# mitrefireline/simfire

Measured on AMD Instinct MI355X. Metric: cell-updates/sec (grid x envs x steps), higher is better.
Workload: dtype u8 status + u8 sprite masks + f64 burn_amounts

## Files before the change

### simfire_amd/csrc/sf_run_kernels.h

```cpp
#pragma once

#include "sf_common.h"
#include "sf_step_kernels.h"

namespace {

constexpr int kMarkDw = 32;
constexpr int kStripDw = 19;
#ifdef SF_NO_PERM_ELIG
#define ELIG(x) elig01(x)
#else
#define ELIG(x) elig01_perm(x)
#endif
constexpr int kRunCtl = 24;
constexpr int kRunMaxD = 4;

typedef uint32_t __attribute__((aligned(1))) u32_unaligned;
typedef uint32_t u32x4 __attribute__((ext_vector_type(4)));

__host__ __device__ inline size_t win_lds_bytes(int n_waves)
{
    const int WR = n_waves * 4;
    return (size_t)WR * 64 * 8 + 8 * 8 * 4 + 128 * 4 + 64 * 4 + (size_t)(WR + 2) * 18 * 4 + (size_t)WR * 16 + (size_t)2 * WR * 64 * 2 + (size_t)2 * WR * 64 +
           (size_t)WR * 64 + (size_t)WR * 8 + 256 * 4;
}
__host__ __device__ inline size_t run_strip_dwords(int n_waves)
{
    const size_t strips = (size_t)n_waves * (64 * kStripDw + kMarkDw), win = (win_lds_bytes(n_waves) + 15) / 16 * 4;
    return strips > win ? strips : win;
}

__host__ __device__ inline size_t run_lds_bytes(const Geo &g, int n_waves, int vcap, int team = 0, int team_rcap = 0)
{
    const int maps = (team || g.VW == 1) ? 4 : 1;
    const int rows = team && team_rcap ? team_rcap + 2 : g.H;
    size_t b = (size_t)maps * rows * g.VW * 8 + (size_t)vcap * 4 + run_strip_dwords(n_waves) * 4 + kRunCtl * 4;
    if (team) b += (size_t)2 * g.PV * 16 + 64 * 4;
#ifdef SF_PHASES
    b += 16 * 16 * 4;
#endif
    return b;
}

}
#include "sf_win_kernels.h"
namespace {

struct RunEnv {
    uint8_t *cells;
    double *burn;
    uint32_t *settled;
    const double *rt;
    unsigned long long *vb;
    unsigned long long *vf, *vl;
    uint8_t *tdirty;
    int32_t *tot;
};

struct WalkCell {
    bool cand;
    uint32_t yx;
    uint32_t own_spost;
    uint32_t owed;
    double bn, r_tab;
};

template <int ATT, int CNT = 0>
__device__ __forceinline__ WalkAcc run_walk(const StepArgs &a, const RunEnv &ev, const Masks &mk, int complete,
                                            uint32_t lo_mask, uint32_t hi_mask, const uint32_t *strips,
                                            uint32_t pend, int lane, int th_log, PhaseClock &pc,
                                            uint32_t excl, uint32_t w16, uint4 s7)
{
    const Geo &g = a.g;
    WalkAcc acc = {0u, 0u, 0u, 0u};
    auto front = [&](uint32_t j, int own) {
        WalkCell c;
        const bool valid = j < pend;
        const int jl = own;
        const uint32_t base = (uint32_t)__builtin_amdgcn_ds_bpermute(jl << 2, (int)excl);
        const uint32_t wl = (uint32_t)__builtin_amdgcn_ds_bpermute(jl << 2, (int)w16);
        int b = 0;
        {
            uint32_t r = valid ? j - base : 0u, x = wl & 0xFFFFu, n;
            n = (uint32_t)__popc(x & 0xFFu); if (r >= n) { r -= n; b += 8; x >>= 8; }
            n = (uint32_t)__popc(x & 0xFu); if (r >= n) { r -= n; b += 4; x >>= 4; }
            n = (uint32_t)__popc(x & 0x3u); if (r >= n) { r -= n; b += 2; x >>= 2; }
            if (r >= (x & 1u)) b += 1;
            b &= 15;
        }
        uint32_t s_post = 0;
        const bool on_line = valid && ((wl >> (16 + b)) & 1u);
        if (__ballot(on_line) != 0ull) {
            const uint32_t d0 = (uint32_t)__builtin_amdgcn_ds_bpermute(jl << 2, (int)s7.x), d1 = (uint32_t)__builtin_amdgcn_ds_bpermute(jl << 2, (int)s7.y);
            const uint32_t d2 = (uint32_t)__builtin_amdgcn_ds_bpermute(jl << 2, (int)s7.z), d3 = (uint32_t)__builtin_amdgcn_ds_bpermute(jl << 2, (int)s7.w);
            const uint32_t dd = (b >> 2) == 0 ? d0 : ((b >> 2) == 1 ? d1 : ((b >> 2) == 2 ? d2 : d3));
            if (on_line) s_post = (dd >> (8 * (b & 3))) & 7u;
        }
        const uint32_t *rec = strips + jl * kStripDw;
        const uint32_t hdr = rec[0];
        const int y = hdr & 0xFFFF, x = (int)(hdr >> 16) * 16 + b;
        const uint32_t idx = (uint32_t)(y * g.P + x);
        const int q = (3 + b) >> 2;
        const uint32_t sh = (uint32_t)(3 + b) & 3u;
        uint32_t u0 = rec[1 + q], u1 = rec[2 + q], m0 = rec[7 + q], m1 = rec[8 + q], d0 = rec[13 + q], d1 = rec[14 + q];
        asm volatile("" : "+v"(u0), "+v"(u1), "+v"(m0), "+v"(m1), "+v"(d0), "+v"(d1));
        const uint32_t up3 = __builtin_amdgcn_alignbyte(u1, u0, sh);
        const uint32_t mid3 = __builtin_amdgcn_alignbyte(m1, m0, sh);
        const uint32_t dn3 = __builtin_amdgcn_alignbyte(d1, d0, sh);
        const int bestk = pick_winner8(up3, mid3, dn3, mk, lo_mask, hi_mask);
        c.cand = valid && bestk >= 0;
        c.yx = (uint32_t)y | ((uint32_t)x << 16);
        c.own_spost = ((mid3 >> 8) & 0xFFu) | (s_post << 8);
        c.owed = 0; c.bn = 0.0; c.r_tab = 0.0;
        {
            const unsigned long long cb = __ballot(c.cand);
            acc.n_active += (uint32_t)__popcll(cb);
            acc.cand |= cb != 0ull;
        }
        if (c.cand) {
            c.bn = ev.burn[idx];
            c.r_tab = ev.rt[(uint32_t)bestk * (uint32_t)(g.H * g.P) + idx];
            if (ATT && s_post >= SF_FIRELINE) c.owed = (uint32_t)complete - ev.settled[idx];
        }
        return c;
    };
    auto back = [&](const WalkCell &c) {
        bool ignited = false;
        if (c.cand) {
            const int y = (int)(c.yx & 0xFFFFu), x = (int)(c.yx >> 16);
            const uint32_t idx = (uint32_t)(y * g.P + x), s_post = c.own_spost >> 8;
            const bool line = s_post >= SF_FIRELINE;
            double bn = c.bn;
            double ros = c.r_tab * g.update_rate;
            if (line) {
                if (ATT) {
                    const double f = line_factor(s_post);
                    bn = lazy_sub(bn, f, c.owed);
                    ros = ros - f;
                    ev.settled[idx] = (uint32_t)complete + 1u;
                } else ros = 0.0;
            }
            bn = bn + ros;
            ev.burn[idx] = bn;
            if (bn > g.pixel_scale) {
                ignited = true;
                const uint8_t nb = (uint8_t)(((c.own_spost & 0xFFu) & ~mk.b_clr) | mk.b_new);
#ifdef SF_STORE_ORDER_WAIT
                asm volatile("s_waitcnt vmcnt(0)" ::: "memory");
#endif
                uint8_t *cell = ev.cells + bl_cell(g, y, x);
                cell[kBlStatus] = (uint8_t)SF_BURNING;
                cell[0] = nb;
                const int bw = y * g.VW + (x >> 10);
                atomicOr(&ev.vb[bw], 1ull << ((x >> 4) & 63));
                if (ev.vf) {
                    if ((x & 15) == 0) atomicOr(&ev.vf[bw], 1ull << ((x >> 4) & 63));
                    if ((x & 15) == 15) atomicOr(&ev.vl[bw], 1ull << ((x >> 4) & 63));
                }
                ev.tdirty[(y >> th_log) * g.TX + ((x >> 4) >> g.logLC)] = 1;
                if (CNT && line) { atomicAdd(ev.tot + s_post, -1); atomicAdd(ev.tot + SF_UNBURNED, 1); }
            }
        }
        acc.n_ignite += (uint32_t)__popcll(__ballot(ignited));
    };
    for (uint32_t j0 = 0; j0 < pend; j0 += 128) {
        const bool two = j0 + 64 < pend;
        int own0 = 0, own1 = 0;
        {
            uint8_t *marks = reinterpret_cast<uint8_t *>(const_cast<uint32_t *>(strips) + 64 * kStripDw);
            reinterpret_cast<uint16_t *>(marks)[lane] = 0;
            const uint32_t mine_n = (uint32_t)__popc(w16 & 0xFFFFu);
            if (mine_n && excl < j0 + 128u && excl + mine_n > j0) marks[excl < j0 ? 0u : excl - j0] = (uint8_t)(lane + 1);
            __builtin_amdgcn_fence(__ATOMIC_RELEASE, "wavefront");
            __builtin_amdgcn_wave_barrier();
            __builtin_amdgcn_fence(__ATOMIC_ACQUIRE, "wavefront");
            const uint32_t m0 = wave_scan_max(marks[lane]);
            own0 = (int)((m0 - 1u) & 63u);
            if (two) {
                const uint32_t carry = wave_last(m0);
                const uint32_t m1 = wave_scan_max(marks[64 + lane]);
                own1 = (int)(((m1 > carry ? m1 : carry) - 1u) & 63u);
            }
        }
        WalkCell c0 = front(j0 + (uint32_t)lane, own0), c1;
        c1.cand = false; c1.yx = 0; c1.own_spost = 0; c1.owed = 0; c1.bn = 0.0; c1.r_tab = 0.0;
        if (two) c1 = front(j0 + 64u + (uint32_t)lane, own1);
        pc.mark(7);
        asm volatile("" : "+v"(c0.bn), "+v"(c0.r_tab), "+v"(c0.owed), "+v"(c1.bn), "+v"(c1.r_tab), "+v"(c1.owed));
        back(c0);
        if (two) back(c1);
        pc.mark(8);
    }
    __builtin_amdgcn_fence(__ATOMIC_RELEASE, "wavefront");
    __builtin_amdgcn_wave_barrier();
    __builtin_amdgcn_fence(__ATOMIC_ACQUIRE, "wavefront");
    pc.mark(9);
    return acc;
}

struct JoinArgs { uint32_t *xj; unsigned long long *xcut; uint32_t *xerr; int E, t_cap, team_recut, join_floor, join_ovh, join_local; unsigned long long team_timeout; };
__device__ __forceinline__ uint4 find_team(const JoinArgs a, uint32_t *sc)
{
    typedef unsigned long long u64;
    const int tid = threadIdx.x, wave = tid >> 6, lane = tid & 63, n_waves = blockDim.x >> 6, nthr = blockDim.x;
    const int E = a.E;
    const uint4 none = make_uint4(0xFFFFFFFFu, 0, 0, 0);
    const uint32_t my_xcc = (uint32_t)__builtin_amdgcn_s_getreg((20 << 0) | (0 << 6) | (31 << 11)) & 15u;
    const unsigned long long t_start = __builtin_amdgcn_s_memrealtime();
    __syncthreads();
    for (;;) {
        uint32_t best = 0, best_e = 0;
        for (int i = tid; i < E; i += nthr) {
            const uint32_t cnt = __hip_atomic_load(a.xj + i, __ATOMIC_RELAXED, __HIP_MEMORY_SCOPE_AGENT);
            const uint32_t b = __hip_atomic_load(a.xj + E + i, __ATOMIC_RELAXED, __HIP_MEMORY_SCOPE_AGENT);
            const long long c = cnt & 0xFFFFu;
            if ((cnt & kJoinClosed) || !b || c >= a.t_cap || c == 0) continue;
            if (a.join_local && __hip_atomic_load(a.xj + 2 * E + 2 + i, __ATOMIC_RELAXED, __HIP_MEMORY_SCOPE_AGENT) != my_xcc) continue;
            const long long per = (long long)(b >> 14) << 4, left = b & 0x3FFFu;
            if (left <= 2 * a.team_recut) continue;
            const long long share_now = per / c, share_join = per / (c + 1);
            const long long now_t = c == 1 ? per : (share_now > a.join_floor ? share_now : a.join_floor) + a.join_ovh;
            const long long join_t = (share_join > a.join_floor ? share_join : a.join_floor) + a.join_ovh;
            if (join_t * 8 >= now_t * 7) continue;
            const long long fin = (now_t * left) >> 8;
            const uint32_t score = fin > 0xFFFFFFFFll ? 0xFFFFFFFFu : (fin < 1 ? 1u : (uint32_t)fin);
            if (score > best) { best = score; best_e = (uint32_t)i; }
        }
        const uint32_t wm = wave_umax(best);
        const int src = __ffsll((long long)__ballot(best == wm)) - 1;
        const uint32_t we = (uint32_t)__builtin_amdgcn_readlane((int)best_e, src);
        if (lane == 0) { sc[wave * 2] = wm; sc[wave * 2 + 1] = we; }
        __syncthreads();
        uint32_t bs = 0, be = 0;
        for (int w = 0; w < n_waves; ++w) { const uint32_t v = sc[2 * w]; if (v > bs) { bs = v; be = sc[2 * w + 1]; } }
        if (tid == 0 && bs == 0) sc[40] = __hip_atomic_load(a.xj + 2 * E, __ATOMIC_RELAXED, __HIP_MEMORY_SCOPE_AGENT);
        __syncthreads();
        if (bs == 0) {
            const uint32_t closed = sc[40];
            __syncthreads();
            if (closed >= (uint32_t)E) return none;
            if (__builtin_amdgcn_s_memrealtime() - t_start > a.team_timeout) return none;
            for (int q = 0; q < 8; ++q) __builtin_amdgcn_s_sleep(127);
            continue;
        }
        if (tid == 0) {
            uint32_t res = 0xFFFFFFFFu;
            const uint32_t old = atomicAdd(a.xj + be, 1u);
            if (!(old & kJoinClosed) && (old & 0xFFFFu) < (uint32_t)a.t_cap) {
                const uint32_t idx = old & 0xFFFFu;
                const unsigned long long t0 = __builtin_amdgcn_s_memrealtime();
                for (;;) {
                    const u64 x = __hip_atomic_load(a.xcut + be, __ATOMIC_RELAXED, __HIP_MEMORY_SCOPE_AGENT);
                    if (x == ~0ull) break;
                    if ((uint32_t)((x >> 24) & 0xFFu) > idx) { res = idx; sc[42] = (uint32_t)((x >> 24) & 0xFFu); sc[43] = (uint32_t)(x & 0xFFFFFFu); break; }
                    __builtin_amdgcn_s_sleep(16);
                    if (__builtin_amdgcn_s_memrealtime() - t0 > a.team_timeout) {
                        *reinterpret_cast<volatile uint32_t *>(a.xerr) = 1u;
                        res = 0xFFFFFFFEu;
                        break;
                    }
                }
            }
            sc[41] = res;
        }
        __syncthreads();
        const uint32_t res = sc[41], tn = sc[42], s0 = sc[43];
        __syncthreads();
        if (res == 0xFFFFFFFEu) return none;
        if (res == 0xFFFFFFFFu) continue;
        __builtin_amdgcn_fence(__ATOMIC_ACQUIRE, "agent");
        return make_uint4(be, res, tn, s0);
    }
}

template <int OFF>
__device__ __forceinline__ uint32_t kernarg_line(const void *ka)
{
    uint32_t d;
    asm volatile("s_load_dword %0, %1, %2" : "=s"(d) : "s"(ka), "n"(OFF));
    return d;
}
template <int BYTES>
__device__ __forceinline__ void kernarg_touch()
{
    const void *ka = (const void *)__builtin_amdgcn_kernarg_segment_ptr();
    uint32_t d0 = 0, d1 = 0, d2 = 0, d3 = 0, d4 = 0, d5 = 0, d6 = 0, d7 = 0, d8 = 0, d9 = 0, d10 = 0, d11 = 0, d12 = 0, d13 = 0, d14 = 0, d15 = 0;
    static_assert(BYTES <= 16 * 64, "more lines than this touches");
    d0 = kernarg_line<0>(ka);
    if (BYTES > 1 * 64) d1 = kernarg_line<1 * 64>(ka);
    if (BYTES > 2 * 64) d2 = kernarg_line<2 * 64>(ka);
    if (BYTES > 3 * 64) d3 = kernarg_line<3 * 64>(ka);
    if (BYTES > 4 * 64) d4 = kernarg_line<4 * 64>(ka);
    if (BYTES > 5 * 64) d5 = kernarg_line<5 * 64>(ka);
    if (BYTES > 6 * 64) d6 = kernarg_line<6 * 64>(ka);
    if (BYTES > 7 * 64) d7 = kernarg_line<7 * 64>(ka);
    if (BYTES > 8 * 64) d8 = kernarg_line<8 * 64>(ka);
    if (BYTES > 9 * 64) d9 = kernarg_line<9 * 64>(ka);
    if (BYTES > 10 * 64) d10 = kernarg_line<10 * 64>(ka);
    if (BYTES > 11 * 64) d11 = kernarg_line<11 * 64>(ka);
    if (BYTES > 12 * 64) d12 = kernarg_line<12 * 64>(ka);
    if (BYTES > 13 * 64) d13 = kernarg_line<13 * 64>(ka);
    if (BYTES > 14 * 64) d14 = kernarg_line<14 * 64>(ka);
    if (BYTES > 15 * 64) d15 = kernarg_line<15 * 64>(ka);
    asm volatile("s_waitcnt lgkmcnt(0)" : "+s"(d0), "+s"(d1), "+s"(d2), "+s"(d3), "+s"(d4), "+s"(d5), "+s"(d6), "+s"(d7), "+s"(d8), "+s"(d9), "+s"(d10), "+s"(d11), "+s"(d12),
                 "+s"(d13), "+s"(d14), "+s"(d15));
}

template <int MAXD, int ATT, int DIAG, int MIT, int TEAM = 0>
__global__ __launch_bounds__(1024) void k_run(StepArgs a_by_value, const int n_steps_launch, int vcap, int bsz)
{
    kernarg_touch<(int)sizeof(StepArgs) + 12>();
#ifdef SF_ARGS_BY_VALUE
    constexpr bool kArgsByValue = true;
#else
    constexpr bool kArgsByValue = TEAM == 2 || MIT == -2 || (MIT == 0 && TEAM == 0) || (TEAM == 1 && MAXD == 2);
#endif
    const StepArgs &a = kArgsByValue ? a_by_value : *(const StepArgs *)__builtin_amdgcn_kernarg_segment_ptr();
    extern __shared__ uint4 s_dyn[];
    const Geo &g = a.g;
    const int tid = threadIdx.x, wave = tid >> 6, lane = tid & 63, n_waves = blockDim.x >> 6, nthr = blockDim.x;
    int e_ = 0, tm_ = 0, tn_ = 1;
    bool no_work = false;
    if (TEAM) {
        const uint32_t tt = a.team_tab[blockIdx.x];
        if (tt == kTeamUnused) { if (TEAM != 2) return; no_work = true; }
        else { e_ = (int)(tt & 0xFFFFu); tm_ = (int)((tt >> 16) & 0xFFu); tn_ = (int)(tt >> 24); }
    } else if (a.todo_cnt) {
        const uint32_t n_left = *a.todo_cnt;
        if (blockIdx.x >= n_left) return;
        e_ = (int)a.todo_list[blockIdx.x];
    } else e_ = a.order ? (int)a.order[blockIdx.x] : (int)blockIdx.x;
    int j_s0 = -1;
    for (bool first_pass = true;; first_pass = false) {
    if (TEAM == 2 && (!first_pass || no_work)) {
        if (a.team_recut >= n_steps_launch) return;
        uint32_t *sc = reinterpret_cast<uint32_t *>(s_dyn);
        JoinArgs ja;
        ja.xj = a.xj; ja.xcut = a.xcut; ja.xerr = a.xerr; ja.E = g.E; ja.team_recut = a.team_recut; ja.join_floor = a.join_floor; ja.join_ovh = a.join_ovh;
        ja.team_timeout = a.team_timeout; ja.join_local = a.join_local; ja.t_cap = kTeamMax < g.TY ? kTeamMax : g.TY;
        const uint4 t = find_team(ja, sc);
        if (t.x == 0xFFFFFFFFu) return;
        e_ = __builtin_amdgcn_readfirstlane((int)t.x); tm_ = __builtin_amdgcn_readfirstlane((int)t.y);
        tn_ = __builtin_amdgcn_readfirstlane((int)t.z); j_s0 = __builtin_amdgcn_readfirstlane((int)t.w);
    }
    {
    int n_steps = n_steps_launch;
    const int e = e_, tm = tm_;
    int tn = tn_;
    const unsigned long long clk0 = __builtin_readcyclecounter();
    const bool fine = TEAM ? true : (MAXD == 1 ? true : g.VW == 1);
    const int VW = MAXD == 1 ? 1 : g.VW;
    const int32_t *const mit = MIT == 0 ? nullptr : a.mit;
    const bool diag = DIAG > 0 ? true : g.diag != 0;
    const int lds_rows = TEAM && a.team_rcap ? a.team_rcap + 2 : g.H;
    unsigned long long *vb0 = reinterpret_cast<unsigned long long *>(s_dyn);
    uint32_t *vlist = reinterpret_cast<uint32_t *>(vb0 + (size_t)(fine ? 4 : 1) * lds_rows * VW);
    uint32_t *strips = vlist + vcap + wave * (64 * kStripDw + kMarkDw);
    uint32_t *ctl = vlist + vcap + run_strip_dwords(n_waves);
#ifdef SF_PHASES
    uint4 *halo = reinterpret_cast<uint4 *>(ctl + kRunCtl + 16 * 16);
#else
    uint4 *halo = reinterpret_cast<uint4 *>(ctl + kRunCtl);
#endif
    uint32_t *tcnt = reinterpret_cast<uint32_t *>(halo + 2 * g.PV);

    constexpr bool kWinPre = (MIT == 0 || MIT == -1) && MAXD == 1 && TEAM == 0;
    constexpr bool kWinAny = ((MIT == 0 && MAXD <= 2) || (MIT == -1 && MAXD == 1 && TEAM == 0 && DIAG == 1)) && TEAM != 2;
    constexpr bool kWinAdvice = kWinAny && !(MAXD == 1 && TEAM == 0);
    unsigned long long pre_w = 0ull, hint_v = 0ull;
    int32_t todo_v = 0;
    EnvState st;
    {
        typedef uint32_t u32x2v __attribute__((ext_vector_type(2)));
        const EnvState *const ps = a.commit + e;
        const bool want_pre = kWinPre && a.win && tid < g.H, want_hint = kWinAdvice && a.win && a.win_hint, want_todo = a.todo != nullptr;
        const void *const p_pre = want_pre ? (const void *)(a.vbits + (long long)e * g.vb_env + tid) : (const void *)ps;
        const void *const p_hint = want_hint ? (const void *)(a.win_hint + e) : (const void *)ps;
        const void *const p_todo = want_todo ? (const void *)(a.todo + e) : (const void *)ps;
        u32x2v v_pre, v_hint, v_hi;
        u32x4 v_lo;
        uint32_t v_todo;
        asm volatile("global_load_dwordx2 %0, %5, off\n\tglobal_load_dwordx2 %1, %6, off\n\tglobal_load_dword %2, %7, off\n\t"
                     "global_load_dwordx4 %3, %8, off\n\tglobal_load_dwordx2 %4, %8, off offset:16\n\ts_waitcnt vmcnt(0)"
                     : "=&v"(v_pre), "=&v"(v_hint), "=&v"(v_todo), "=&v"(v_lo), "=&v"(v_hi)
                     : "v"(p_pre), "v"(p_hint), "v"(p_todo), "v"(ps)
                     : "memory");
        if (want_pre) pre_w = (unsigned long long)v_pre.x | ((unsigned long long)v_pre.y << 32);
        if (want_hint) hint_v = (unsigned long long)v_hint.x | ((unsigned long long)v_hint.y << 32);
        if (want_todo) todo_v = (int32_t)v_todo;
        st.running = __builtin_amdgcn_readfirstlane((int)v_lo.x); st.steps = __builtin_amdgcn_readfirstlane((int)v_lo.y);
        st.complete = __builtin_amdgcn_readfirstlane((int)v_lo.z); st.time_quit = __builtin_amdgcn_readfirstlane((int)v_lo.w);
        st.elapsed = __hiloint2double(__builtin_amdgcn_readfirstlane((int)v_hi.y), __builtin_amdgcn_readfirstlane((int)v_hi.x));
    }
    const unsigned long long hint_pre = (unsigned long long)(uint32_t)__builtin_amdgcn_readfirstlane((int)(uint32_t)hint_v) | ((unsigned long long)(uint32_t)__builtin_amdgcn_readfirstlane((int)(uint32_t)(hint_v >> 32)) << 32);
    if (a.todo) n_steps = __builtin_amdgcn_readfirstlane(todo_v);
    if ((!st.running && !mit) || n_steps < 0) n_steps = 0;
    if (!TEAM && a.todo && a.todo_skip && n_steps == 0) return;
    unsigned long long *vb_glob = a.vbits + (long long)e * g.vb_env;
    const int n_words = g.H * VW;
    if (tid < kRunCtl) ctl[tid] = 0;
    const int th_log = 31 - __builtin_clz((unsigned)(g.LR * g.RB));
    uint32_t n_active = 0, n_ignite = 0, n_items_acc = 0, n_phase2 = 0, n_vec_done = 0;
    constexpr bool kWin = ((MIT == 0 && MAXD <= 2) || (MIT == -1 && MAXD == 1 && TEAM == 0 && DIAG == 1)) && TEAM != 2;
    constexpr int kWinGen = (MAXD == 1 && TEAM == 0) ? 0 : 1;
    constexpr int kWinMit = MIT == -1 ? 1 : 0;
    int32_t px = 0, py = 0, pty = 0;
    int s_begin = 0;
    bool win_result = false;
    PhaseClock wpc;
    const bool win_mit_ok = !kWinMit || !mit || a.mit_k <= 64;
    if (kWinMit && mit && a.mit_k <= 64 && n_steps > 0 && wave == n_waves - 1 && lane < a.mit_k) {
        const int32_t *p0 = mit + ((long long)e * a.mit_k + lane) * 3;
        px = p0[0]; py = p0[1]; pty = p0[2];
    }
    if (kWin && (!TEAM || tn == 1) && win_mit_ok && j_s0 < 0) {
        WinEnv we;
        we.cells = a.cells + (long long)e * g.cells_env;
        we.burn = a.burn + (long long)e * g.plane_env;
        we.settled = a.settled ? a.settled + (long long)e * g.plane_env : nullptr;
        we.rtc = a.rtc ? a.rtc + (long long)e * g.rt_env : nullptr;
        we.tdirty = a.tdirty + (long long)e * g.TY * g.TX;
        we.thist = a.thist + (long long)e * g.TY * g.TX * 8;
        we.vb_glob = vb_glob;
        we.vb_plane = (long long)g.E * g.vb_env;
        wpc.start();
#ifdef SF_PHASES
        wpc.tl = (e == g_timeline_env && g_timeline_step == -1) ? g_timeline + wave * 64 : nullptr;
#endif
        wpc.note(30);
        we.pre_w = pre_w; we.pre = kWinPre; we.hint = hint_pre;
        s_begin = run_window<ATT, kWinGen, kWinMit>(a, we, st, n_steps, diag, vlist + vcap, ctl, th_log, n_active, n_ignite, n_vec_done, wpc, e, win_result,
                                                    kWinMit ? mit : nullptr, n_steps, &px, &py, &pty, vlist, vcap >= 1024 ? 15 : 11);
        if (a.counters && tid == 0 && s_begin)
            atomicAdd(a.counters + (size_t)((blockIdx.x * 16) & (kCounterShards - 1)) * kCounterRow + 8, (unsigned long long)s_begin);
    }
    if (TEAM == 2 && j_s0 >= 0) s_begin = j_s0;
    const bool general = !kWin || (TEAM && tn > 1) || (s_begin < n_steps && (st.running || mit));
    if (TEAM == 0 && kWin && MIT == 0 && !general) {
#ifdef SF_PHASES
        if (lane == 0 && g_wave_log_launch == -2 && e < 4096) {
            if (wave == 0) { g_wave_log[e * 4 + 0] = __builtin_readcyclecounter() - clk0; g_wave_log[e * 4 + 2] = (unsigned long long)st.steps; }
            atomicAdd(&g_wave_log[e * 4 + 1], (unsigned long long)n_vec_done);
        }
#endif
        wpc.note(35);
        if (tid == 0) {
            a.commit[e] = st;
            if (a.cost) {
                const unsigned long long c = (__builtin_readcyclecounter() - clk0) >> 4;
                a.cost[e] = c > 0x0FFFFFFFull ? 0x0FFFFFFFu : (uint32_t)c;
            }
        }
        wpc.note(49);
        if (a.counters && lane == 0) {
            unsigned long long *cs = a.counters + (size_t)((blockIdx.x * 16 + wave) & (kCounterShards - 1)) * kCounterRow;
            if (n_active) atomicAdd(&cs[0], (unsigned long long)n_active);
            if (n_ignite) atomicAdd(&cs[1], (unsigned long long)n_ignite);
            if (n_vec_done) atomicAdd(&cs[5], (unsigned long long)n_vec_done);
        }
        if (a.res_block && !win_result && !(a.row_valid && n_steps == 0 && !mit)) {
            __syncthreads();
            counts_env(g, e, a.status, a.cells, a.tdirty, a.thist, st.running, st.steps, st.elapsed, a.res_block, a.res_elapsed, a.res_sink,
                       reinterpret_cast<int32_t (*)[6]>(vlist + vcap));
        }
        return;
    }
    int R0 = 0, R1 = g.H;
    auto cut_bands = [&](int steps_ahead) -> bool {
        int tid = threadIdx.x;
        asm volatile("" : "+v"(tid));
        const int lane = tid & 63, wave = tid >> 6;
        const int th = g.LR * g.RB, ntr = (g.H + th - 1) / th;
        if (tid < 64) tcnt[tid] = 0;
        __syncthreads();
        for (int y = tid; y < g.H; y += nthr) {
            uint32_t c = 0;
            for (int w = 0; w < VW; ++w) c += (uint32_t)__popcll(vb_glob[y * VW + w]);
            if (c) atomicAdd(&tcnt[y / th], c);
        }
        __syncthreads();
        if (wave == 0) {
            const uint32_t ci = lane < ntr ? tcnt[lane] : 0u;
            const uint32_t incl = wave_scan_incl(ci, lane), total = wave_last(incl);
            const unsigned long long nzb = __ballot(ci != 0u);
            int lo = 0, hi = ntr;
            if (a.team_rcap && nzb && !mit) {
                const int mt = (steps_ahead + 1 + th - 1) / th + 1;
                lo = __ffsll((long long)nzb) - 1 - mt; hi = 64 - __clzll((long long)nzb) + mt;
                lo = lo < 0 ? 0 : lo; hi = hi > ntr ? ntr : hi;
                if (hi - lo < tn) { hi = lo + tn < ntr ? lo + tn : ntr; lo = hi - tn > 0 ? hi - tn : 0; }
            }
            const int cap = a.team_rcap ? a.team_rcap / th : ntr;
            if (a.team_rcap && !nzb && !mit) hi = ntr < cap * tn ? ntr : cap * tn;
            int cut[kTeamMax + 1];
            cut[0] = lo; cut[tn] = hi;
            for (int j = 1; j < tn; ++j) {
                const unsigned long long bal = __ballot(lane < ntr && (unsigned long long)incl * (unsigned)tn >= (unsigned long long)total * (unsigned)j);
                int c = total ? __ffsll((long long)bal) : lo + (hi - lo) * j / tn;
                if (c < cut[j - 1] + 1) c = cut[j - 1] + 1;
                if (c > cut[j - 1] + cap) c = cut[j - 1] + cap;
                cut[j] = c;
            }
            for (int j = tn - 1; j >= 1; --j) {
                if (cut[j] > cut[j + 1] - 1) cut[j] = cut[j + 1] - 1;
                if (cut[j] < cut[j + 1] - cap) cut[j] = cut[j + 1] - cap;
            }
            bool fits = true;
            for (int j = 0; j < tn; ++j) fits = fits && cut[j + 1] - cut[j] >= 1 && cut[j + 1] - cut[j] <= cap;
            if (lane == 0) { tcnt[0] = (uint32_t)(cut[tm] * th); tcnt[1] = (uint32_t)(cut[tm + 1] * th); tcnt[2] = fits ? 1u : 0u; }
        }
        __syncthreads();
        R0 = (int)tcnt[0]; R1 = (int)tcnt[1];
        const bool fits = __builtin_amdgcn_readfirstlane((int)tcnt[2]) != 0;
        R0 = __builtin_amdgcn_readfirstlane(R0); R1 = __builtin_amdgcn_readfirstlane(R1);
        if (R1 > g.H) R1 = g.H;
        __syncthreads();
        return fits;
    };
    {
        bool fits = true;
        if (TEAM && (tn > 1 || a.team_rcap) && general) fits = cut_bands(tn > 1 && a.team_recut > 0 && a.team_recut < n_steps ? a.team_recut : n_steps - s_begin);
        if (TEAM && a.todo_out && tm == 0 && tid == 0) a.todo_out[e] = fits ? 0 : n_steps - s_begin;
        if (TEAM && !fits) {
            if (!a.todo_out && tid == 0) *reinterpret_cast<volatile uint32_t *>(a.xerr) = 1u;
            if (s_begin > 0 && tm == 0 && tid == 0) a.commit[e] = st;
            return;
        }
    }
    bool has_up = TEAM && tm > 0, has_dn = TEAM && tm + 1 < tn;
    if (TEAM == 2 && tm == 0 && j_s0 < 0 && tid == 0)
        __hip_atomic_store(a.xj + 2 * g.E + 2 + e, (uint32_t)__builtin_amdgcn_s_getreg((20 << 0) | (0 << 6) | (31 << 11)) & 15u, __ATOMIC_RELAXED, __HIP_MEMORY_SCOPE_AGENT);
    auto team_release = [&]() {
        if (TEAM == 2 && a.join_local == 1) asm volatile("s_waitcnt vmcnt(0)" ::: "memory");
        else __builtin_amdgcn_fence(__ATOMIC_RELEASE, "agent");
    };
    auto team_acquire = [&]() { __builtin_amdgcn_fence(__ATOMIC_ACQUIRE, "agent"); };
    bool one_l2 = false;
    bool gave_up = false;
    auto line_up = [&](const uint32_t tag, const bool report) {
        typedef unsigned long long u64;
        int lane = threadIdx.x & 63;
        asm volatile("" : "+v"(lane));
        const uint32_t xcc = (uint32_t)__builtin_amdgcn_s_getreg((20 << 0) | (0 << 6) | (31 << 11)) & 15u;
        if (lane == 0) __hip_atomic_store(a.xg + ((size_t)e * kTeamMax + tm) * 3 + 2, ((u64)tag << 32) | (u64)xcc, __ATOMIC_RELAXED, __HIP_MEMORY_SCOPE_AGENT);
        u64 x = ((u64)tag << 32) | xcc;
        const unsigned long long t0 = __builtin_amdgcn_s_memrealtime();
        for (;;) {
            if (lane < tn) x = __hip_atomic_load(a.xg + ((size_t)e * kTeamMax + lane) * 3 + 2, __ATOMIC_RELAXED, __HIP_MEMORY_SCOPE_AGENT);
            if (__all((uint32_t)(x >> 32) >= tag)) break;
            __builtin_amdgcn_s_sleep(2);
            if (gave_up || __builtin_amdgcn_s_memrealtime() - t0 > a.team_timeout) {
                if (report) {
                    if (lane == 0) *reinterpret_cast<volatile uint32_t *>(a.xerr) = 1u;
                    gave_up = true;
                }
                break;
            }
        }
        one_l2 = __all((uint32_t)(x >> 32) >= tag && ((uint32_t)x & 15u) == xcc) && !a.team_far;
    };
    unsigned long long *vb = vb0, *vf = nullptr, *vl = nullptr, *ve = nullptr;
    auto load_band = [&]() {
        int tid = threadIdx.x;
        asm volatile("" : "+v"(tid));
        const int yoff = TEAM && a.team_rcap ? R0 - 1 : 0;
        vb = vb0 - (long long)yoff * VW;
        vf = fine ? vb + (size_t)lds_rows * VW : nullptr; vl = fine ? vb + (size_t)2 * lds_rows * VW : nullptr;
        ve = fine ? vb + (size_t)3 * lds_rows * VW : nullptr;
        const int y_lo = TEAM && a.team_rcap ? (R0 > 0 ? R0 - 1 : 0) : 0, y_hi = TEAM && a.team_rcap ? (R1 < g.H ? R1 + 1 : g.H) : g.H;
        for (int i = y_lo * VW + tid; i < y_hi * VW; i += nthr) {
            vb[i] = vb_glob[i];
            if (fine) {
                vf[i] = vb_glob[(long long)g.E * g.vb_env + i];
                vl[i] = vb_glob[2ll * g.E * g.vb_env + i];
                ve[i] = ~0ull;
            }
        }
        if (TEAM && tn > 1) {
            for (int i = tid; i < 2 * g.PV; i += nthr) {
                const int side = i >= g.PV, v = side ? i - g.PV : i, yh = side ? R1 : R0 - 1;
                uint4 r = make_uint4(0, 0, 0, 0);
                if (side ? has_dn : has_up)
                    r = *reinterpret_cast<const uint4 *>(a.cells + (long long)e * g.cells_env + bl_vec(g, yh, v) + (yh & 1) * 16);
                halo[i] = r;
            }
        }
    };
    if (general) load_band();
    PhaseClock pc;
#ifdef SF_PHASES
    uint32_t *ph_acc = ctl + kRunCtl + wave * 16;
    if (lane < 16) ph_acc[lane] = 0;
    pc.start(ph_acc);
#else
    pc.start();
#endif
    __syncthreads();
    if (TEAM == 1 && tn > 1) {
        if (tid == 0) {
            uint32_t *w = a.xdone + g.E + e;
            constexpr uint32_t kGo = 0x40000000u, kAbort = 0x80000000u, kDecided = 0xC0000000u;
            auto decide = [&](uint32_t bit) -> uint32_t {
                for (;;) {
                    uint32_t cur = __hip_atomic_load(w, __ATOMIC_RELAXED, __HIP_MEMORY_SCOPE_AGENT);
                    if (cur & kDecided) return cur & kDecided;
                    if (__hip_atomic_compare_exchange_strong(w, &cur, cur | bit, __ATOMIC_RELAXED, __ATOMIC_RELAXED, __HIP_MEMORY_SCOPE_AGENT)) return bit;
                }
            };
            const uint32_t mine = __hip_atomic_fetch_add(w, 1u, __ATOMIC_RELAXED, __HIP_MEMORY_SCOPE_AGENT) + 1u;
            uint32_t d = mine & kDecided;
            if (!d && (mine & 0xFFFFu) == (uint32_t)tn) d = decide(kGo);
            if (!d && a.team_start_timeout == 0ull) d = decide(kAbort);
            const unsigned long long t0 = __builtin_amdgcn_s_memrealtime();
            while (!d) {
                d = __hip_atomic_load(w, __ATOMIC_RELAXED, __HIP_MEMORY_SCOPE_AGENT) & kDecided;
                if (d) break;
                __builtin_amdgcn_s_sleep(8);
                if (__builtin_amdgcn_s_memrealtime() - t0 >= a.team_start_timeout) d = decide(kAbort);
            }
            ctl[16] = d == kGo ? 1u : 2u;
            if (d != kGo && tm == 0) __hip_atomic_fetch_add(a.xdone + 2 * g.E, 1u, __ATOMIC_RELAXED, __HIP_MEMORY_SCOPE_AGENT);
        }
        __syncthreads();
        if (__builtin_amdgcn_readfirstlane((int)ctl[16]) != 1) {
            if (tm != 0) return;
            tn = 1;
            has_up = false; has_dn = false;
            bool fits = true;
            if (a.team_rcap) fits = cut_bands(n_steps - s_begin);
            else { R0 = 0; R1 = g.H; }
            if (a.todo_out && tid == 0) a.todo_out[e] = fits ? 0 : n_steps - s_begin;
            if (!fits) {
                if (!a.todo_out && tid == 0) *reinterpret_cast<volatile uint32_t *>(a.xerr) = 1u;
                return;
            }
            __syncthreads();
            load_band();
            __syncthreads();
        }
    }
    if (TEAM && tn > 1) {
        if (wave == 0) line_up(TEAM == 2 && j_s0 >= 0 ? 2u + (uint32_t)(j_s0 / a.team_recut) : 1u, TEAM == 2 && j_s0 >= 0);
        if (TEAM == 2) __syncthreads();
    }

    RunEnv ev;
    ev.cells = a.cells + (long long)e * g.cells_env;
    ev.burn = a.burn + (long long)e * g.plane_env;
    ev.settled = a.settled ? a.settled + (long long)e * g.plane_env : nullptr;
    ev.rt = a.rt + (long long)e * g.rt_env;
    ev.vb = vb; ev.vf = vf; ev.vl = vl;
    ev.tdirty = a.tdirty + (long long)e * g.TY * g.TX;
    ev.tot = reinterpret_cast<int32_t *>(ctl + 10);
    int rpt = ((TEAM ? R1 - R0 : g.H) + nthr - 1) / nthr;
    int row0 = TEAM ? R0 : 0;
    auto store_band = [&]() {
        int tid = threadIdx.x;
        asm volatile("" : "+v"(tid));
        for (int i = R0 * VW + tid; i < R1 * VW; i += nthr) {
            vb_glob[i] = vb[i];
            vb_glob[(long long)g.E * g.vb_env + i] = vf[i];
            vb_glob[2ll * g.E * g.vb_env + i] = vl[i];
        }
    };
    const unsigned long long last_word_mask = (g.PV & 63) ? ((1ull << (g.PV & 63)) - 1ull) : ~0ull;

    const bool mit_one_wave = mit && a.mit_k <= 64;
    const int mit_wave = n_waves - 1;
    constexpr bool loop = MIT == -2;
    auto load_pt = [&](int s) {
        if (wave == mit_wave && lane < a.mit_k) {
            const int32_t *p = mit + (((long long)s * g.E + e) * a.mit_k + lane) * 3;
            px = p[0]; py = p[1]; pty = p[2];
        }
    };
    if (mit_one_wave && n_steps > 0 && !loop && !kWinMit) load_pt(0);
    uint32_t lseq = 0;
    if (loop) {
        if (tid == 0) ctl[18] = __hip_atomic_load(a.loop_done + e, __ATOMIC_RELAXED, __HIP_MEMORY_SCOPE_AGENT);
        __syncthreads();
        lseq = (uint32_t)__builtin_amdgcn_readfirstlane((int)ctl[18]);
        n_steps = 0x7FFFFFFF;
        counts_env(g, e, a.status, a.cells, a.tdirty, a.thist, st.running, st.steps, st.elapsed, a.res_block, a.res_elapsed, nullptr,
                   reinterpret_cast<int32_t (*)[6]>(vlist + vcap));
        if (tid == 0)
            for (int q = 0; q < 6; ++q) ev.tot[q] = a.res_block[e * 8 + 2 + q];
        if (e == 0 && a.mit_k > 0 && lseq > 0) {
            const int n16 = g.E * a.mit_k;
            const u32x4 *src = reinterpret_cast<const u32x4 *>(a.loop_pts_host) + (size_t)(lseq & 1u) * n16;
            u32x4 *cpy = reinterpret_cast<u32x4 *>(a.loop_pts) + (size_t)(lseq & 1u) * n16;
            for (int i = tid; i < n16; i += nthr) {
                u32x4 v;
                asm volatile("global_load_dwordx4 %0, %1, off sc0 sc1\n\ts_waitcnt vmcnt(0)" : "=&v"(v) : "v"(src + i) : "memory");
                if (v.w == lseq) asm volatile("global_store_dwordx4 %0, %1, off sc0 sc1" :: "v"(cpy + i), "v"(v) : "memory");
            }
        }
        __syncthreads();
    }
    unsigned long long join_clk = __builtin_readcyclecounter();
    unsigned long long x_clocks = 0;
    uint32_t x_steps = 0;
    for (int s = s_begin; s < n_steps && (st.running || mit); ++s) {
        const int k = s % 3, kn = (s + 1) % 3;
#ifdef SF_PHASES
        pc.tl = (e == g_timeline_env && s == g_timeline_step) ? g_timeline + wave * 64 : nullptr;
#endif
        auto loop_finish = [&]() {
            __syncthreads();
            if (tid == 0) {
                const int32_t *tot = ev.tot;
                int32_t *row = a.res_block + e * 8;
                row[0] = st.running == 1; row[1] = st.steps;
                for (int q = 0; q < 6; ++q) row[2 + q] = tot[q];
                a.res_elapsed[e] = st.elapsed;
            }
            ++lseq;
            if (wave == 0) {
                uint32_t *stage = strips;
                if (lane == 0) {
                    const int32_t *row = a.res_block + e * 8;
                    const unsigned long long el = (unsigned long long)__double_as_longlong(st.elapsed);
                    stage[0] = (uint32_t)row[0]; stage[1] = (uint32_t)row[1]; stage[2] = (uint32_t)row[2];
                    stage[4] = (uint32_t)row[3]; stage[5] = (uint32_t)row[4]; stage[6] = (uint32_t)row[5];
                    stage[8] = (uint32_t)row[6]; stage[9] = (uint32_t)row[7]; stage[10] = (uint32_t)el;
                    stage[12] = (uint32_t)(el >> 32); stage[13] = 0u; stage[14] = 0u;
                    stage[3] = stage[7] = stage[11] = stage[15] = lseq;
                    __hip_atomic_store(a.loop_done + e, lseq, __ATOMIC_RELAXED, __HIP_MEMORY_SCOPE_AGENT);
                }
                __builtin_amdgcn_fence(__ATOMIC_RELEASE, "wavefront");
                __builtin_amdgcn_wave_barrier();
                __builtin_amdgcn_fence(__ATOMIC_ACQUIRE, "wavefront");
                if (lane < 16)
                    __hip_atomic_store(reinterpret_cast<uint32_t *>(a.loop_res_host) + (size_t)e * 16 + lane, stage[lane], __ATOMIC_RELAXED, __HIP_MEMORY_SCOPE_SYSTEM);
            }
        };
        if (loop && a.mit_k > 0) {
            const uint32_t want = lseq + 1u;
            const int n16 = g.E * a.mit_k;
            const u32x4 *src = reinterpret_cast<const u32x4 *>(a.loop_pts_host) + (size_t)(want & 1u) * n16;
            u32x4 *cpy = reinterpret_cast<u32x4 *>(a.loop_pts) + (size_t)(want & 1u) * n16;
            if (e == 0) {
                volatile uint32_t *flag = ctl + 19;
                uint32_t db = 0;
                if (wave < (n_waves >= 8 ? 4 : 1)) {
                    const unsigned long long t0 = __builtin_readcyclecounter();
                    if (wave) __builtin_amdgcn_s_sleep(1);
                    for (int it = 0;; ++it) {
                        db = *flag;
                        if (db) break;
                        if (it == 0 && wave == 1) __builtin_amdgcn_s_sleep(20);
                        if (it == 0 && wave == 2) __builtin_amdgcn_s_sleep(40);
                        if (it == 0 && wave == 3) __builtin_amdgcn_s_sleep(60);
                        db = __hip_atomic_load(a.loop_db, __ATOMIC_RELAXED, __HIP_MEMORY_SCOPE_SYSTEM);
                        if (!((db & ~kLoopStop) > lseq || (db & kLoopStop))) {
                            if (__builtin_readcyclecounter() - t0 <= a.loop_timeout) { __builtin_amdgcn_s_sleep(4); continue; }
                            db = lseq | kLoopStop;
                        }
                        if (lane == 0) atomicCAS(ctl + 19, 0u, db);
                        db = *flag;
                        break;
                    }
                } else {
                    while ((db = *flag) == 0u) __builtin_amdgcn_s_sleep(1);
                }
                db = (uint32_t)__builtin_amdgcn_readfirstlane((int)db);
                if ((db & ~kLoopStop) > lseq) {
                    for (;;) {
                        uint32_t c = lane == 0 ? atomicAdd(ctl + 21, 1u) : 0u;
                        c = (uint32_t)__builtin_amdgcn_readfirstlane((int)c);
                        const int i0 = (int)c * 256 + lane;
                        if ((int)c * 256 >= n16) break;
                        const int i1 = i0 + 64, i2 = i0 + 128, i3 = i0 + 192, last = n16 - 1;
                        u32x4 v0, v1, v2, v3;
                        asm volatile("global_load_dwordx4 %0, %4, off sc0 sc1\n\tglobal_load_dwordx4 %1, %5, off sc0 sc1\n\t"
                                     "global_load_dwordx4 %2, %6, off sc0 sc1\n\tglobal_load_dwordx4 %3, %7, off sc0 sc1\n\ts_waitcnt vmcnt(0)"
                                     : "=&v"(v0), "=&v"(v1), "=&v"(v2), "=&v"(v3)
                                     : "v"(src + (i0 < last ? i0 : last)), "v"(src + (i1 < last ? i1 : last)), "v"(src + (i2 < last ? i2 : last)), "v"(src + (i3 < last ? i3 : last))
                                     : "memory");
                        if (i0 < n16) asm volatile("global_store_dwordx4 %0, %1, off sc1" :: "v"(cpy + i0), "v"(v0) : "memory");
                        if (i1 < n16) asm volatile("global_store_dwordx4 %0, %1, off sc1" :: "v"(cpy + i1), "v"(v1) : "memory");
                        if (i2 < n16) asm volatile("global_store_dwordx4 %0, %1, off sc1" :: "v"(cpy + i2), "v"(v2) : "memory");
                        if (i3 < n16) asm volatile("global_store_dwordx4 %0, %1, off sc1" :: "v"(cpy + i3), "v"(v3) : "memory");
                    }
                } else if (tid == 0) {
                    __hip_atomic_store(a.loop_seq, lseq | kLoopStop, __ATOMIC_RELAXED, __HIP_MEMORY_SCOPE_AGENT);
                }
            }
            if (wave == mit_wave) {
                const u32x4 *mine = cpy + (size_t)e * a.mit_k + (lane < a.mit_k ? lane : 0);
                const unsigned long long t0 = __builtin_readcyclecounter();
                uint32_t go = 0;
                for (;;) {
                    u32x4 v;
                    uint32_t q;
                    asm volatile("global_load_dwordx4 %0, %2, off sc1\n\tglobal_load_dword %1, %3, off sc1\n\ts_waitcnt vmcnt(0)"
                                 : "=&v"(v), "=&v"(q) : "v"(mine), "v"(a.loop_seq) : "memory");
                    if (__ballot(lane < a.mit_k && v.w != want) == 0ull) { go = 1; px = (int32_t)v.x; py = (int32_t)v.y; pty = (int32_t)v.z; break; }
                    if ((q & kLoopStop) || __builtin_readcyclecounter() - t0 > 2 * a.loop_timeout) break;
                    __builtin_amdgcn_s_sleep(2);
                }
                if (lane == 0) ctl[17] = go;
            }
            __syncthreads();
            if (!ctl[17]) break;
            if (e == 0 && tid == 0) { ctl[19] = 0; ctl[21] = 0; }
        } else if (loop) {
            if (e == 0) {
                if (tid == 0) {
                    const unsigned long long t0 = __builtin_readcyclecounter();
                    uint32_t db;
                    for (;;) {
                        db = __hip_atomic_load(a.loop_db, __ATOMIC_RELAXED, __HIP_MEMORY_SCOPE_SYSTEM);
                        if ((db & ~kLoopStop) > lseq || (db & kLoopStop)) break;
                        if (__builtin_readcyclecounter() - t0 > a.loop_timeout) { db = lseq | kLoopStop; break; }
                        __builtin_amdgcn_s_sleep(4);
                    }
                    ctl[19] = db;
                }
                __syncthreads();
                const uint32_t db = ctl[19];
                __syncthreads();
                if (tid == 0) __hip_atomic_store(a.loop_seq, db, __ATOMIC_RELAXED, __HIP_MEMORY_SCOPE_AGENT);
            }
            if (tid == 0) {
                const unsigned long long t0 = __builtin_readcyclecounter();
                uint32_t go = 0;
                for (;;) {
                    const uint32_t q = __hip_atomic_load(a.loop_seq, __ATOMIC_RELAXED, __HIP_MEMORY_SCOPE_AGENT);
                    if ((q & ~kLoopStop) > lseq) { go = 1; break; }
                    if ((q & kLoopStop) || __builtin_readcyclecounter() - t0 > 2 * a.loop_timeout) break;
                    __builtin_amdgcn_s_sleep(2);
                }
                ctl[17] = go;
            }
            __syncthreads();
            if (!ctl[17]) break;
        }
        if (mit) {
            if (mit_one_wave) {
                bool ok = false;
                int x = 0, y = 0;
                if (wave == mit_wave) {
                    const int ty = pty;
                    ok = lane < a.mit_k && ty >= SF_FIRELINE && ty <= SF_WETLINE && px >= 0 && px < g.W && py >= R0 && py < R1;
                    x = ok ? px : 0;
                    y = ok ? py : R0;
                    if (ok && fine) atomicOr(&ve[y * VW + (x >> 10)], 1ull << ((x >> 4) & 63));
                }
                __builtin_amdgcn_fence(__ATOMIC_RELEASE, "workgroup", "local");
                __builtin_amdgcn_s_barrier();
                __builtin_amdgcn_fence(__ATOMIC_ACQUIRE, "workgroup", "local");
                pc.mark(13);
                if (wave == mit_wave) {
                    const int ty = pty;
                    const uint32_t o = (uint32_t)(y * g.P + x);
                    uint8_t *cell = ev.cells + bl_cell(g, y, x & ~3) + kBlStatus + (x & 3);
                    if (s + 1 < n_steps && !loop) load_pt(s + 1);
                    uint32_t was = 0, owed_since = 0;
                    double bn = 0.0;
                    if (ATT && ok) { was = *cell & 7u; bn = ev.burn[o]; owed_since = ev.settled[o]; }
                    else if (loop && ok) was = *cell & 7u;
                    int fin = ty;
                    bool first = ok;
                    const unsigned long long above = loop ? __ballot(ok) : __ballot(ok && ty > SF_FIRELINE);
                    if (above && (loop || __ballot(ok && ty != SF_WETLINE) != 0ull)) {
                        const uint32_t h = (o * 2654435761u) >> 17, bit = 1u << (h & 31);
                        if (ok) strips[h >> 5] = 0;
                        __builtin_amdgcn_fence(__ATOMIC_RELEASE, "wavefront");
                        __builtin_amdgcn_wave_barrier();
                        __builtin_amdgcn_fence(__ATOMIC_ACQUIRE, "wavefront");
                        const uint32_t clash = ok ? (atomicOr(&strips[h >> 5], bit) & bit) : 0u;
                        if (__ballot(clash != 0) != 0ull) {
                            const uint32_t key = ok ? o : 0xFFFFFFFFu;
                            for (unsigned long long hi = above; hi; hi &= hi - 1) {
                                const int j = __ffsll((long long)hi) - 1;
                                const uint32_t kj = (uint32_t)__builtin_amdgcn_readlane((int)key, j);
                                const int tj = __builtin_amdgcn_readlane(ty, j);
                                if (key == kj && tj > fin) fin = tj;
                                if (loop && key == kj && j < lane) first = false;
                            }
                        }
                    }
                    if (ATT && ok && was != (uint32_t)fin) {
                        if (was >= SF_FIRELINE) ev.burn[o] = lazy_sub(bn, line_factor(was), (uint32_t)st.complete - owed_since);
                        ev.settled[o] = (uint32_t)st.complete;
                    }
                    if (ok) *cell = (uint8_t)fin;
                    if (ok) ev.tdirty[(y >> th_log) * g.TX + ((x >> 4) >> g.logLC)] = 1;
                    if (loop && first && was != (uint32_t)fin) { atomicAdd(ev.tot + was, -1); atomicAdd(ev.tot + fin, 1); }
                    pc.mark(14);
                }
            } else {
                int tid = threadIdx.x;
                asm volatile("" : "+v"(tid));
                const int32_t *pts = mit + ((long long)s * g.E + e) * a.mit_k * 3;
                for (int i = tid; i < a.mit_k; i += nthr) {
                    const int x = pts[3 * i], y = pts[3 * i + 1], ty = pts[3 * i + 2];
                    if (ty < SF_FIRELINE || ty > SF_WETLINE || x < 0 || x >= g.W || y < R0 || y >= R1) continue;
                    const uint32_t o = (uint32_t)(y * g.P + x);
                    uint32_t *word = reinterpret_cast<uint32_t *>(ev.cells + bl_cell(g, y, x & ~3) + kBlStatus);
                    const int sh = (x & 3) * 8;
                    const uint32_t old = (atomicAnd(word, ~(0xFFu << sh)) >> sh) & 7u;
                    if (ATT && old >= SF_FIRELINE) ev.burn[o] = lazy_sub(ev.burn[o], line_factor(old), (uint32_t)st.complete - ev.settled[o]);
                }
                __syncthreads();
                for (int i = tid; i < a.mit_k; i += nthr) {
                    const int x = pts[3 * i], y = pts[3 * i + 1], ty = pts[3 * i + 2];
                    if (ty < SF_FIRELINE || ty > SF_WETLINE || x < 0 || x >= g.W || y < R0 || y >= R1) continue;
                    const uint32_t o = (uint32_t)(y * g.P + x);
                    uint32_t *word = reinterpret_cast<uint32_t *>(ev.cells + bl_cell(g, y, x & ~3) + kBlStatus);
                    const int sh = (x & 3) * 8;
                    uint32_t old = *word, seen;
                    do {
                        seen = old;
                        if (((seen >> sh) & 0xFFu) >= (uint32_t)ty) break;
                        old = atomicCAS(word, seen, (seen & ~(0xFFu << sh)) | ((uint32_t)ty << sh));
                    } while (old != seen);
                    if (ATT) ev.settled[o] = (uint32_t)st.complete;
                    ev.tdirty[(y >> th_log) * g.TX + ((x >> 4) >> g.logLC)] = 1;
                    if (fine) atomicOr(&ve[y * VW + (x >> 10)], 1ull << ((x >> 4) & 63));
                }
                __syncthreads();
            }
            if (!st.running) {
                if (loop) loop_finish();
                continue;
            }
        }
        pc.mark(15);
        if (tid < 3) ctl[3 * tid + kn] = 0;
        const int t = st.steps + 1;
        const Masks mk = make_masks(t, g.md, g.N);
        const bool spread = !st.time_quit;
        const uint32_t L4 = rep4(mk.m_live), EXP4 = rep4(mk.b_exp), CLR4 = rep4(mk.b_clr);
        const int exp_sh = __ffs(mk.b_exp) - 1;
        const uint32_t lo_mask = diag ? L4 : (L4 & 0xFF00FF00u), hi_mask = diag ? L4 : (L4 & 0x00FF00FFu);

        unsigned long long D[MAXD];
        uint32_t cnt = 0;
        if (fine) {
#pragma unroll
            for (int d = 0; d < MAXD; ++d) {
                D[d] = 0;
                const int i = MAXD == 1 ? 0 : d / VW, w = MAXD == 1 ? 0 : d - i * VW;
                const int y = row0 + tid * rpt + i;
                if (i < rpt && y < R1) {
                    int o = y * VW + w;
                    asm volatile("" : "+v"(o));
                    const int up_o = y > 0 ? -VW : 0, dn_o = y + 1 < g.H ? VW : 0;
                    const unsigned long long b1 = vb[o], l1 = vl[o], f1 = vf[o], e1 = ve[o];
                    unsigned long long b02 = 0, l02 = 0, f02 = 0;
                    if (up_o) { b02 = vb[o + up_o]; l02 = vl[o + up_o]; f02 = vf[o + up_o]; }
                    if (dn_o) { b02 |= vb[o + dn_o]; l02 |= vl[o + dn_o]; f02 |= vf[o + dn_o]; }
                    unsigned long long edge = ((l02 | l1) << 1) | ((f02 | f1) >> 1);
                    if (MAXD > 1 && VW > 1) {
                        if (w > 0) edge |= (vl[o - 1] | vl[o - 1 + up_o] | vl[o - 1 + dn_o]) >> 63;
                        if (w + 1 < VW) edge |= (vf[o + 1] | vf[o + 1 + up_o] | vf[o + 1 + dn_o]) << 63;
                    }
                    unsigned long long m = b1 | (e1 & (b02 | edge)) | l02 | f02;
                    if (g.dense) m = ~0ull;
                    if (w == VW - 1) m &= last_word_mask;
                    D[d] = m;
                    cnt += (uint32_t)__popcll(m);
                }
            }
        } else {
#pragma unroll
            for (int d = 0; d < MAXD; ++d) {
                D[d] = 0;
                const int i = d / g.VW, w = d - i * g.VW;
                const int y = tid * rpt + i;
                if (i < rpt && y < g.H) {
                    const unsigned long long *row = vb + y * g.VW;
                    const int up_o = y > 0 ? -g.VW : 0, dn_o = y + 1 < g.H ? g.VW : 0;
                    unsigned long long m = row[w] | row[w + up_o] | row[w + dn_o];
                    m |= (m << 1) | (m >> 1);
                    if (w > 0) m |= (row[w - 1] | row[w - 1 + up_o] | row[w - 1 + dn_o]) >> 63;
                    if (w + 1 < g.VW) m |= (row[w + 1] | row[w + 1 + up_o] | row[w + 1 + dn_o]) << 63;
                    if (g.dense) m = ~0ull;
                    if (w == g.VW - 1) m &= last_word_mask;
                    D[d] = m;
                    cnt += (uint32_t)__popcll(m);
                }
            }
        }
        uint32_t pos0 = 0;
#ifndef SF_NO_SKIP_EMPTY
        if (__ballot(cnt != 0) != 0ull)
#endif
        {
            const uint32_t incl = wave_scan_incl(cnt, lane);
            const uint32_t wave_total = wave_last(incl);
            uint32_t wbase = 0;
            if (lane == 0) wbase = atomicAdd(&ctl[k], wave_total);
            wbase = (uint32_t)__builtin_amdgcn_readfirstlane((int)wbase);
            pos0 = wbase + incl - cnt;
        }
        pc.mark(1);

        uint32_t n_all = 0;
        for (uint32_t cb = 0;; cb += (uint32_t)vcap) {
            {
                uint32_t p = pos0;
#pragma unroll
                for (int d = 0; d < MAXD; ++d) {
                    const unsigned long long m = D[d];
                    const int i = d / g.VW, w = d - i * g.VW;
                    const uint32_t base_item = (uint32_t)(row0 + tid * rpt + i) | ((uint32_t)(w * 64) << 16);
                    uint32_t lo = (uint32_t)m, hi = (uint32_t)(m >> 32);
                    while (lo) {
                        const uint32_t b = (uint32_t)__ffs(lo) - 1u;
                        lo &= lo - 1;
                        const uint32_t slot = p - cb;
                        if (slot < (uint32_t)vcap) vlist[slot] = base_item + (b << 16);
                        p++;
                    }
                    while (hi) {
                        const uint32_t b = (uint32_t)__ffs(hi) + 31u;
                        hi &= hi - 1;
                        const uint32_t slot = p - cb;
                        if (slot < (uint32_t)vcap) vlist[slot] = base_item + (b << 16);
                        p++;
                    }
                }
            }
            __syncthreads();
            n_all = ctl[k];
            const uint32_t n_chunk = n_all - cb < (uint32_t)vcap ? n_all - cb : (uint32_t)vcap;
            pc.mark(2);

            struct VecIn { uint32_t item; uint4 up, mid, dn, sr; uint32_t l0, l1, l2, r0, r1, r2; };
            const bool dealt = n_waves == 16 && n_chunk <= 2u * (uint32_t)bsz;
            auto grab = [&]() {
                uint32_t j = 0;
                if (lane == 0) j = atomicAdd(&ctl[6 + k], (uint32_t)bsz);
                return (uint32_t)__builtin_amdgcn_readfirstlane((int)j) + (dealt ? (uint32_t)(n_waves * bsz) : 0u);
            };
            auto fetch = [&](uint32_t j0, VecIn &in) {
                const bool has = lane < bsz && j0 + lane < n_chunk;
                const uint32_t item = vlist[has ? j0 + lane : n_chunk - 1];
                const int y = item & 0xFFFF, v = (item >> 16) & 0xFF;
                const int x0 = v * 16;
                const int odd = y & 1;
                const uint8_t *sec = ev.cells + bl_vec(g, y, v);
                const uint8_t *p_mid = sec + odd * 16, *p_pair = sec + (odd ^ 1) * 16;
                const uint8_t *p_far = ev.cells + bl_vec(g, odd ? y + 1 : y - 1, v) + (odd ^ 1) * 16;
                const uint8_t *p_up = odd ? p_pair : p_far, *p_dn = odd ? p_far : p_pair;
                in.item = has ? item : 0xFFFFFFFFu;
                in.mid = *reinterpret_cast<const uint4 *>(p_mid);
                in.sr = *reinterpret_cast<const uint4 *>(p_mid + kBlStatus);
                in.up = *reinterpret_cast<const uint4 *>(p_up);
                in.dn = *reinterpret_cast<const uint4 *>(p_dn);
                in.l0 = in.l1 = in.l2 = in.r0 = in.r1 = in.r2 = 0;
                if (has && lane == 0 && v > 0) {
                    in.l0 = *reinterpret_cast<const uint32_t *>(p_mid - 128 + 12);
                    if (diag) { in.l1 = *reinterpret_cast<const uint32_t *>(p_up - 128 + 12); in.l2 = *reinterpret_cast<const uint32_t *>(p_dn - 128 + 12); }
                }
                if (has && (j0 + lane + 1 == n_chunk || lane == bsz - 1) && x0 + 16 < g.W) {
                    in.r0 = *reinterpret_cast<const uint32_t *>(p_mid + 128);
                    if (diag) { in.r1 = *reinterpret_cast<const uint32_t *>(p_up + 128); in.r2 = *reinterpret_cast<const uint32_t *>(p_dn + 128); }
                }
            };
            const uint32_t j_first = dealt ? (uint32_t)(wave * bsz) : grab();
            pc.note(16);
            VecIn vin_a, vin_b;
            if (j_first < n_chunk) fetch(j_first, vin_a);
            pc.note(17);
            auto batch = [&](const VecIn &cur, const uint32_t j0, VecIn &nxt, uint32_t &j_next) __attribute__((always_inline)) {
                j_next = j0 + (uint32_t)bsz < n_chunk ? grab() : n_chunk;
                pc.note(18);
                constexpr bool kEarly = !(TEAM && MAXD == 2);
                if (kEarly && j_next < n_chunk) fetch(j_next, nxt);
#ifdef SF_PHASES
                pc.mark(3);
                asm volatile("" :: "v"(cur.mid.x), "v"(cur.sr.x), "v"(cur.up.x), "v"(cur.dn.x));
                pc.mark(11);
#endif
                const bool has = cur.item != 0xFFFFFFFFu;
                const uint32_t item = cur.item;
                const int y = item & 0xFFFF, v = (item >> 16) & 0xFF;
                const int x0 = v * 16;
                const uint32_t voff = (uint32_t)(y * g.P + x0);
                uint8_t *vmask = ev.cells + bl_vec(g, y, v) + (y & 1) * 16;
                const uint4 mid = cur.mid, sr = cur.sr;
                uint4 up = cur.up, dn = cur.dn;
                uint32_t cl1 = cur.l1, cl2 = cur.l2, cr1 = cur.r1, cr2 = cur.r2;
                const bool last_lane = j0 + lane + 1 == n_chunk || lane == bsz - 1;
                if (TEAM) {
                    const bool hu = has_up && y == R0, hd = has_dn && y == R1 - 1;
                    if (hu | hd) {
                        const uint4 *hrow = halo + (hd ? g.PV : 0);
                        const uint4 hv = hrow[v];
                        if (hu) up = hv; else dn = hv;
                        if (diag) {
                            if (lane == 0 && v > 0) { const uint32_t q = hrow[v - 1].w; if (hu) cl1 = q; else cl2 = q; }
                            if (last_lane && x0 + 16 < g.W) { const uint32_t q = hrow[v + 1].x; if (hu) cr1 = q; else cr2 = q; }
                        }
                    }
                }
                const uint32_t item_l = (uint32_t)__builtin_amdgcn_update_dpp(-1, (int)item, 0x138, 0xF, 0xF, false);
                const uint32_t item_r = (uint32_t)__builtin_amdgcn_update_dpp(-1, (int)item, 0x130, 0xF, 0xF, false);
                n_vec_done += (lane == 0) ? (n_chunk - j0 < (uint32_t)bsz ? n_chunk - j0 : (uint32_t)bsz) : 0u;
                const uint4 midL = and4(mid, L4);
                const uint4 vsrc = and4(or4(up, dn), L4);
                const uint4 hsrc = diag ? or4(midL, vsrc) : midL;
                uint32_t l0 = cur.l0 & 0xFF000000u, l1 = cl1 & 0xFF000000u, l2 = cl2 & 0xFF000000u;
                uint32_t r0 = cur.r0 & 0xFFu, r1 = cr1 & 0xFFu, r2 = cr2 & 0xFFu;
                {
                    const uint32_t dl0 = (uint32_t)__builtin_amdgcn_update_dpp(0, (int)mid.w, 0x138, 0xF, 0xF, false);
                    const uint32_t dl1 = (uint32_t)__builtin_amdgcn_update_dpp(0, (int)up.w, 0x138, 0xF, 0xF, false);
                    const uint32_t dl2 = (uint32_t)__builtin_amdgcn_update_dpp(0, (int)dn.w, 0x138, 0xF, 0xF, false);
                    const uint32_t dr0 = (uint32_t)__builtin_amdgcn_update_dpp(0, (int)mid.x, 0x130, 0xF, 0xF, false);
                    const uint32_t dr1 = (uint32_t)__builtin_amdgcn_update_dpp(0, (int)up.x, 0x130, 0xF, 0xF, false);
                    const uint32_t dr2 = (uint32_t)__builtin_amdgcn_update_dpp(0, (int)dn.x, 0x130, 0xF, 0xF, false);
                    if (lane != 0 && item_l + 0x10000u == item) { l0 = dl0 & 0xFF000000u; l1 = dl1 & 0xFF000000u; l2 = dl2 & 0xFF000000u; }
                    if (!last_lane && item_r == item + 0x10000u) { r0 = dr0 & 0xFFu; r1 = dr1 & 0xFFu; r2 = dr2 & 0xFFu; }
                }
                uint32_t lin = (diag ? (l0 | l1 | l2) : l0) >> 24, rin = diag ? (r0 | r1 | r2) : r0;
                if (has) {
                    uint32_t *rec = strips + lane * kStripDw;
                    rec[0] = item & 0x00FFFFFFu;
                    rec[1] = l1; rec[2] = up.x; rec[3] = up.y; rec[4] = up.z; rec[5] = up.w; rec[6] = r1;
                    rec[7] = l0; rec[8] = mid.x; rec[9] = mid.y; rec[10] = mid.z; rec[11] = mid.w; rec[12] = r0;
                    rec[13] = l2; rec[14] = dn.x; rec[15] = dn.y; rec[16] = dn.z; rec[17] = dn.w; rec[18] = r2;
                }
                lin &= mk.m_live;
                rin &= mk.m_live;
                if (__ballot(has && any4(midL) != 0) != 0ull && lane == 0) reinterpret_cast<uint8_t *>(ctl + 3 + k)[0] = 1;
                uint4 nb;
                nb.x = vsrc.x | ((hsrc.x << 8) | lin) | __builtin_amdgcn_alignbyte(hsrc.y, hsrc.x, 1);
                nb.y = vsrc.y | __builtin_amdgcn_alignbyte(hsrc.y, hsrc.x, 3) | __builtin_amdgcn_alignbyte(hsrc.z, hsrc.y, 1);
                nb.z = vsrc.z | __builtin_amdgcn_alignbyte(hsrc.z, hsrc.y, 3) | __builtin_amdgcn_alignbyte(hsrc.w, hsrc.z, 1);
                nb.w = vsrc.w | __builtin_amdgcn_alignbyte(hsrc.w, hsrc.z, 3) | ((hsrc.w >> 8) | (rin << 24));
                pc.mark(4);

                const uint4 ex4 = and4(mid, EXP4);
                const uint32_t any_exp = any4(ex4), any_clr = any4(and4(mid, CLR4)), any_nb = spread ? any4(nb) : 0u;
                if (has && any_clr) {
                    const uint4 av = and4(mid, ~CLR4);
                    *reinterpret_cast<uint4 *>(vmask) = av;
                    if (!any4(av)) atomicAnd(&vb[y * VW + (v >> 6)], ~(1ull << (v & 63)));
                    if (fine) {
                        if (!(av.x & 0xFFu) && (mid.x & 0xFFu)) atomicAnd(&vf[y * VW + (v >> 6)], ~(1ull << (v & 63)));
                        if (!(av.w >> 24) && (mid.w >> 24)) atomicAnd(&vl[y * VW + (v >> 6)], ~(1ull << (v & 63)));
                    }
                }
                uint32_t m16 = 0;
                uint4 snew = sr;
                if (has && (any_exp | any_nb)) {
                    const uint4 s7 = and4(sr, 0x07070707u);
                    uint4 em;
                    em.x = spread01((ex4.x >> exp_sh) & 0x01010101u);
                    em.y = spread01((ex4.y >> exp_sh) & 0x01010101u);
                    em.z = spread01((ex4.z >> exp_sh) & 0x01010101u);
                    em.w = spread01((ex4.w >> exp_sh) & 0x01010101u);
                    snew.x = (s7.x & ~em.x) | (0x02020202u & em.x);
                    snew.y = (s7.y & ~em.y) | (0x02020202u & em.y);
                    snew.z = (s7.z & ~em.z) | (0x02020202u & em.z);
                    snew.w = (s7.w & ~em.w) | (0x02020202u & em.w);
                    if ((snew.x ^ sr.x) | (snew.y ^ sr.y) | (snew.z ^ sr.z) | (snew.w ^ sr.w)) {
                        *reinterpret_cast<uint4 *>(vmask + kBlStatus) = snew;
                        if (ATT) {
                            uint32_t sp16 = pack4(ge3_01(s7.x) & em.x & 0x01010101u) | (pack4(ge3_01(s7.y) & em.y & 0x01010101u) << 4) |
                                            (pack4(ge3_01(s7.z) & em.z & 0x01010101u) << 8) | (pack4(ge3_01(s7.w) & em.w & 0x01010101u) << 12);
                            while (sp16) {
                                const int b = __ffs(sp16) - 1;
                                sp16 &= sp16 - 1;
                                const uint32_t s_pre = (pick(s7, b >> 2) >> (8 * (b & 3))) & 7u;
                                ev.burn[voff + b] = lazy_sub(ev.burn[voff + b], line_factor(s_pre), (uint32_t)st.complete - ev.settled[voff + b]);
                            }
                        }
                    }
                    if (any_nb) {
                        uint32_t p0 = ELIG(snew.x) & nz01(nb.x);
                        uint32_t p1 = ELIG(snew.y) & nz01(nb.y);
                        uint32_t p2 = ELIG(snew.z) & nz01(nb.z);
                        uint32_t p3 = ELIG(snew.w) & nz01(nb.w);
                        if (__builtin_expect(x0 + 16 > g.W, 0)) {
                            const int nv = g.W - x0;
                            p0 &= first01(nv); p1 &= first01(nv - 4); p2 &= first01(nv - 8); p3 &= first01(nv - 12);
                        }
                        m16 = pack4(p0) | (pack4(p1) << 4) | (pack4(p2) << 8) | (pack4(p3) << 12);
                    }
                }
                if (fine && has) {
                    uint32_t el = ELIG(snew.x) | ELIG(snew.y) |
                                  ELIG(snew.z) | ELIG(snew.w);
                    if (__builtin_expect(x0 + 16 > g.W, 0)) {
                        const int nv = g.W - x0;
                        el = (ELIG(snew.x) & first01(nv)) | (ELIG(snew.y) & first01(nv - 4)) |
                             (ELIG(snew.z) & first01(nv - 8)) | (ELIG(snew.w) & first01(nv - 12));
                    }
                    if (!el) atomicAnd(&ve[y * VW + (v >> 6)], ~(1ull << (v & 63)));
                }
                const bool st_ch = ((snew.x ^ sr.x) | (snew.y ^ sr.y) | (snew.z ^ sr.z) | (snew.w ^ sr.w)) != 0;
                if (st_ch) ev.tdirty[(y >> th_log) * g.TX + (v >> g.logLC)] = 1;
                if (loop && st_ch) {
                    const uint4 s7o = and4(sr, 0x07070707u);
                    const uint32_t wo[4] = {s7o.x, s7o.y, s7o.z, s7o.w}, wn[4] = {snew.x & 0x07070707u, snew.y & 0x07070707u, snew.z & 0x07070707u, snew.w & 0x07070707u};
                    int n = 0;
#pragma unroll
                    for (int j = 0; j < 4; ++j)
                        for (uint32_t ch = nz01(wo[j] ^ wn[j]); ch; ch &= ch - 1) {
                            atomicAdd(ev.tot + ((wo[j] >> (__ffs(ch) - 1)) & 7u), -1);
                            ++n;
                        }
                    if (n) atomicAdd(ev.tot + SF_BURNED, n);
                }
                pc.mark(5);

                const uint32_t mine = (uint32_t)__popc(m16);
                if (__ballot(mine != 0) != 0ull) {
                    const uint32_t incl_c = wave_scan_incl(mine, lane);
                    const uint32_t total = wave_last(incl_c);
                    const uint32_t excl = incl_c - mine;
                    const uint4 s7n = and4(snew, 0x07070707u);
                    uint32_t line16 = 0;
                    if (__ballot((((s7n.x | s7n.y | s7n.z | s7n.w) + 0x05050505u) & 0x08080808u) != 0) != 0ull)
                        line16 = pack4(ge3_01(s7n.x)) | (pack4(ge3_01(s7n.y)) << 4) | (pack4(ge3_01(s7n.z)) << 8) | (pack4(ge3_01(s7n.w)) << 12);
                    __builtin_amdgcn_fence(__ATOMIC_RELEASE, "wavefront");
                    __builtin_amdgcn_wave_barrier();
                    __builtin_amdgcn_fence(__ATOMIC_ACQUIRE, "wavefront");
                    pc.mark(6);
                    const WalkAcc wk = run_walk<ATT, loop ? 1 : 0>(a, ev, mk, st.complete, lo_mask, hi_mask, strips, total, lane, th_log, pc, excl, m16 | (line16 << 16), s7n);
                    n_active += wk.n_active;
                    n_ignite += wk.n_ignite;
                    if (loop && wk.n_ignite && lane == 0) { atomicAdd(ev.tot + SF_UNBURNED, -(int32_t)wk.n_ignite); atomicAdd(ev.tot + SF_BURNING, (int32_t)wk.n_ignite); }
                    if (wk.cand && lane == 0) reinterpret_cast<uint8_t *>(ctl + 3 + k)[1] = 1;
                    n_items_acc += (lane == 0) ? total : 0u;
                    n_phase2++;
                } else {
                    __builtin_amdgcn_wave_barrier();
                }
                pc.mark(10);
                if (!kEarly && j_next < n_chunk) fetch(j_next, nxt);
            };
            if (TEAM == 0 && MAXD == 1) {
                for (uint32_t ja = j_first; ja < n_chunk;) {
                    uint32_t jb;
                    batch(vin_a, ja, vin_b, jb);
                    if (jb >= n_chunk) break;
                    batch(vin_b, jb, vin_a, ja);
                }
            } else {
                for (uint32_t ja = j_first; ja < n_chunk;) {
                    const VecIn cur = vin_a;
                    const uint32_t j0 = ja;
                    batch(cur, j0, vin_a, ja);
                }
            }
            if (cb + (uint32_t)vcap >= n_all) break;
            __syncthreads();
            if (tid == 0) ctl[6 + k] = 0;
        }
        if (TEAM && tn > 1) asm volatile("s_waitcnt vmcnt(0)" ::: "memory");
        __syncthreads();
        pc.mark(0);
        const bool cut_step = TEAM && a.team_recut > 0 && (s + 1) % a.team_recut == 0 && s + 1 < n_steps;
        const bool recut_now = cut_step && tn > 1;
        int tn_new = tn;
        if (TEAM == 2 && cut_step) {
            if (tm == 0 && tid == 0) {
                const uint32_t c = __hip_atomic_load(a.xj + e, __ATOMIC_RELAXED, __HIP_MEMORY_SCOPE_AGENT) & 0xFFu;
                const uint32_t t_cap = (uint32_t)(kTeamMax < g.TY ? kTeamMax : g.TY);
                ctl[20] = c > t_cap ? t_cap : (c < (uint32_t)tn ? (uint32_t)tn : c);
                const unsigned long long now = __builtin_readcyclecounter();
                long long per = (long long)((now - join_clk) / (unsigned long long)a.team_recut);
                join_clk = now;
                if (tn > 1) per = (per - a.join_ovh) * tn;
                if (per < a.join_floor) per = a.join_floor;
                const long long left = n_steps - (s + 1);
                const uint32_t b = (uint32_t)((per >> 4) > 0x3FFFF ? 0x3FFFF : (per >> 4)) << 14 | (uint32_t)(left > 0x3FFF ? 0x3FFF : left);
                __hip_atomic_store(a.xj + g.E + e, b, __ATOMIC_RELAXED, __HIP_MEMORY_SCOPE_AGENT);
            }
            if (!recut_now) __syncthreads();
        }
        if (recut_now) {
            store_band();
            team_release();
            __syncthreads();
        }
        if (TEAM == 2 && cut_step && tm == 0) tn_new = __builtin_amdgcn_readfirstlane((int)ctl[20]);
        if (TEAM && tn > 1) {
            if (wave == 0) {
                typedef unsigned long long u64;
                int lane = threadIdx.x & 63;
                asm volatile("" : "+v"(lane));
                const unsigned long long xt0 = a.counters ? __builtin_readcyclecounter() : 0ull;
                const uint32_t epoch = (uint32_t)s + 1u, par = (uint32_t)s & 1u;
                uint8_t *xb_me = a.xbuf + ((size_t)(e * kTeamMax + tm) * 4) * (size_t)a.xrow;
                for (int side = 0; side < 2 && !one_l2; ++side) {
                    if (!(side ? has_dn : has_up)) continue;
                    const int yb = side ? R1 - 1 : R0;
                    u64 *dst = reinterpret_cast<u64 *>(xb_me + (size_t)(side * 2 + par) * a.xrow);
                    for (int v = lane; v < g.PV; v += 64)
                        if ((vb[yb * VW + (v >> 6)] >> (v & 63)) & 1ull) {
                            const uint4 val = *reinterpret_cast<const uint4 *>(ev.cells + bl_vec(g, yb, v) + (yb & 1) * 16);
                            if (one_l2) *reinterpret_cast<uint4 *>(dst + 8 + v * 2) = val;
                            else {
                                __hip_atomic_store(dst + 8 + v * 2, (u64)val.x | ((u64)val.y << 32), __ATOMIC_RELAXED, __HIP_MEMORY_SCOPE_AGENT);
                                __hip_atomic_store(dst + 8 + v * 2 + 1, (u64)val.z | ((u64)val.w << 32), __ATOMIC_RELAXED, __HIP_MEMORY_SCOPE_AGENT);
                            }
                        }
                    if (lane < 3 * VW) {
                        const int which = lane / VW, w = lane - which * VW;
                        const u64 word = (which == 0 ? vb : (which == 1 ? vf : vl))[yb * VW + w];
                        if (one_l2) __hip_atomic_store(dst + lane, word, __ATOMIC_RELAXED, __HIP_MEMORY_SCOPE_WORKGROUP);
                        else __hip_atomic_store(dst + lane, word, __ATOMIC_RELAXED, __HIP_MEMORY_SCOPE_AGENT);
                    }
                }
                asm volatile("s_waitcnt vmcnt(0)" ::: "memory");
                if (lane == 0) {
                    const u64 gv = ((u64)epoch << 32) | (u64)(ctl[3 + k] & 0xFFFFu) | (TEAM == 2 ? (u64)tn_new << 16 : 0ull);
                    if (one_l2) __hip_atomic_store(a.xg + ((size_t)e * kTeamMax + tm) * 3 + par, gv, __ATOMIC_RELAXED, __HIP_MEMORY_SCOPE_WORKGROUP);
                    else __hip_atomic_store(a.xg + ((size_t)e * kTeamMax + tm) * 3 + par, gv, __ATOMIC_RELAXED, __HIP_MEMORY_SCOPE_AGENT);
                }
                u64 x = (u64)epoch << 32;
                {
                    const unsigned long long t0 = __builtin_amdgcn_s_memrealtime();
                    for (;;) {
                        if (lane < tn) x = __hip_atomic_load(a.xg + ((size_t)e * kTeamMax + lane) * 3 + par, __ATOMIC_RELAXED, __HIP_MEMORY_SCOPE_AGENT);
                        if (__all((uint32_t)(x >> 32) == epoch)) break;
                        __builtin_amdgcn_s_sleep(1);
                        if (gave_up || __builtin_amdgcn_s_memrealtime() - t0 > a.team_timeout) {
                            if (lane == 0) *reinterpret_cast<volatile uint32_t *>(a.xerr) = 1u;
                            gave_up = true;
                            break;
                        }
                    }
                }
                const bool live_any = __ballot(lane < tn && (x & 0xFFull)) != 0ull, cand_any = __ballot(lane < tn && (x & 0xFF00ull)) != 0ull;
                if (lane == 0) ctl[3 + k] = (live_any ? FLAG_LIVE : 0u) | (cand_any ? FLAG_CAND : 0u);
                if (TEAM == 2 && cut_step && lane == 0) ctl[20] = (uint32_t)(x >> 16) & 0xFFu;
                for (int side = 0; side < 2 && one_l2; ++side) {
                    if (!(side ? has_dn : has_up)) continue;
                    const int yh = side ? R1 : R0 - 1;
                    for (int v0 = 0; v0 < g.PV; v0 += 64) {
                        const int v = v0 + lane;
                        u64 lo = 0, hi = 0;
                        if (v < g.PV) {
                            const u64 *src = reinterpret_cast<const u64 *>(ev.cells + bl_vec(g, yh, v) + (yh & 1) * 16);
                            lo = __hip_atomic_load(src, __ATOMIC_RELAXED, __HIP_MEMORY_SCOPE_AGENT);
                            hi = __hip_atomic_load(src + 1, __ATOMIC_RELAXED, __HIP_MEMORY_SCOPE_AGENT);
                        }
                        if (v < g.PV) halo[side * g.PV + v] = make_uint4((uint32_t)lo, (uint32_t)(lo >> 32), (uint32_t)hi, (uint32_t)(hi >> 32));
                        const u64 bw = __ballot((lo | hi) != 0ull), fw = __ballot((lo & 0xFFull) != 0ull), lw = __ballot((hi >> 56) != 0ull);
                        if (lane == 0) { vb[yh * VW + (v0 >> 6)] = bw; vf[yh * VW + (v0 >> 6)] = fw; vl[yh * VW + (v0 >> 6)] = lw; }
                    }
                }
                for (int side = 0; side < 2 && !one_l2; ++side) {
                    if (!(side ? has_dn : has_up)) continue;
                    const int nj = side ? tm + 1 : tm - 1, yh = side ? R1 : R0 - 1;
                    const u64 *src = reinterpret_cast<const u64 *>(a.xbuf + ((size_t)(e * kTeamMax + nj) * 4 + (size_t)((side ^ 1) * 2 + par)) * a.xrow);
                    u64 word = 0;
                    if (lane < 3 * VW) word = __hip_atomic_load(src + lane, __ATOMIC_RELAXED, __HIP_MEMORY_SCOPE_AGENT);
                    for (int v0 = 0; v0 < g.PV; v0 += 64) {
                        const int v = v0 + lane;
                        u64 lo = 0, hi = 0;
                        if (v < g.PV) {
                            lo = __hip_atomic_load(src + 8 + v * 2, __ATOMIC_RELAXED, __HIP_MEMORY_SCOPE_AGENT);
                            hi = __hip_atomic_load(src + 8 + v * 2 + 1, __ATOMIC_RELAXED, __HIP_MEMORY_SCOPE_AGENT);
                        }
                        const int wl = v0 >> 6;
                        const u64 bw = (u64)(uint32_t)__builtin_amdgcn_readlane((int)(uint32_t)word, wl) |
                                       ((u64)(uint32_t)__builtin_amdgcn_readlane((int)(uint32_t)(word >> 32), wl) << 32);
                        if (v < g.PV) {
                            const bool on = (bw >> lane) & 1ull;
                            halo[side * g.PV + v] = on ? make_uint4((uint32_t)lo, (uint32_t)(lo >> 32), (uint32_t)hi, (uint32_t)(hi >> 32)) : make_uint4(0, 0, 0, 0);
                        }
                    }
                    if (lane < 3 * VW) {
                        const int which = lane / VW, w = lane - which * VW;
                        (which == 0 ? vb : (which == 1 ? vf : vl))[yh * VW + w] = word;
                    }
                }
                if (a.counters && lane == 0) { x_clocks += __builtin_readcyclecounter() - xt0; x_steps++; }
            }
            __builtin_amdgcn_fence(__ATOMIC_RELEASE, "workgroup", "local");
            __builtin_amdgcn_s_barrier();
            __builtin_amdgcn_fence(__ATOMIC_ACQUIRE, "workgroup", "local");
        }
        st = fold_state(st, ctl[3 + k], g);
        st.running = __builtin_amdgcn_readfirstlane(st.running);
        st.steps = __builtin_amdgcn_readfirstlane(st.steps);
        st.complete = __builtin_amdgcn_readfirstlane(st.complete);
        st.time_quit = __builtin_amdgcn_readfirstlane(st.time_quit);
        if (loop) loop_finish();
        if (TEAM == 2 && cut_step && tn > 1) tn_new = __builtin_amdgcn_readfirstlane((int)ctl[20]);
        if (TEAM == 2 && gave_up) tn_new = tn;
        if ((recut_now || tn_new > tn) && (st.running || mit)) {
            if (TEAM == 2 && tn == 1) {
                store_band();
                team_release();
                __syncthreads();
            }
            if (TEAM == 2 && tn_new > tn && tm == 0 && tid == 0) {
                a.commit[e] = st;
                team_release();
                __hip_atomic_store(a.xcut + e, ((unsigned long long)tn_new << 24) | (unsigned long long)(s + 1), __ATOMIC_RELAXED, __HIP_MEMORY_SCOPE_AGENT);
                atomicAdd(a.xj + 2 * g.E + 1, (uint32_t)(tn_new - tn));
                const uint32_t li = atomicAdd(a.jlog, 1u);
                if (li < (uint32_t)kJoinLog) { a.jlog[1 + 3 * li] = (uint32_t)e; a.jlog[2 + 3 * li] = (uint32_t)(s + 1); a.jlog[3 + 3 * li] = (uint32_t)tn_new; }
            }
            team_acquire();
            if (TEAM == 2) { tn = tn_new; has_up = tm > 0; has_dn = tm + 1 < tn; }
            const int left = n_steps - (s + 1);
            cut_bands(a.team_recut < left ? a.team_recut : left);
            load_band();
            ev.vb = vb; ev.vf = vf; ev.vl = vl;
            rpt = (R1 - R0 + nthr - 1) / nthr;
            row0 = R0;
            __syncthreads();
            if (wave == 0) line_up(2u + (uint32_t)((s + 1) / a.team_recut), true);
            __syncthreads();
        }
    }
    if (TEAM == 2 && tm == 0 && tid == 0) {
        atomicOr(a.xj + e, kJoinClosed);
        __hip_atomic_store(a.xcut + e, ~0ull, __ATOMIC_RELAXED, __HIP_MEMORY_SCOPE_AGENT);
        __hip_atomic_store(a.xj + g.E + e, 0u, __ATOMIC_RELAXED, __HIP_MEMORY_SCOPE_AGENT);
        atomicAdd(a.xj + 2 * g.E, 1u);
        a.tsize[e] = (uint32_t)tn;
        const uint32_t li = atomicAdd(a.jlog, 1u);
        if (li < (uint32_t)kJoinLog) { a.jlog[1 + 3 * li] = (uint32_t)e; a.jlog[2 + 3 * li] = (uint32_t)__builtin_amdgcn_s_memrealtime(); a.jlog[3 + 3 * li] = 0xFFu; }
    }
#ifdef SF_PHASES
    pc.mark(12);
    if (lane == 0 && g_wave_log_launch == -2)
        for (int q = 0; q < 16; ++q) if (pc.acc[q]) atomicAdd(&g_phase[q], (unsigned long long)pc.acc[q]);
    if (lane == 0 && g_wave_log_launch == -2 && e < 4096) {
        if (wave == 0) { g_wave_log[e * 4 + 0] = __builtin_readcyclecounter() - pc.t0; g_wave_log[e * 4 + 2] = (unsigned long long)st.steps; }
        atomicAdd(&g_wave_log[e * 4 + 1], (unsigned long long)n_vec_done);
    }
#endif
    wpc.note(35);
    if (general) __syncthreads();
    if (tid == 0) {
        if (!TEAM || tm == 0) a.commit[e] = st;
        if (kWinAdvice && general && a.win_hint && (!TEAM || tm == 0)) a.win_hint[e] = 0ull;
        if (a.cost) {
            const unsigned long long c = (__builtin_readcyclecounter() - clk0) >> 4;
            const uint32_t c32 = c > 0x0FFFFFFFull ? 0x0FFFFFFFu : (uint32_t)c;
            if (TEAM && tn > 1) atomicAdd(&a.cost[e], c32);
            else a.cost[e] = c32;
        }
    }
    if (TEAM) {
        if (general) store_band();
    } else if (general) {
        for (int i = tid; i < n_words; i += nthr) vb_glob[i] = vb[i];
        if (fine)
            for (int i = tid; i < g.H; i += nthr) {
                vb_glob[(long long)g.E * g.vb_env + i] = vf[i];
                vb_glob[2ll * g.E * g.vb_env + i] = vl[i];
            }
    }
    wpc.note(49);
    if (a.counters && lane == 0) {
        int cw = wave;
        asm volatile("" : "+v"(cw));
        unsigned long long *cs = a.counters + (size_t)((blockIdx.x * 16 + cw) & (kCounterShards - 1)) * kCounterRow;
        if (n_active) atomicAdd(&cs[0], (unsigned long long)n_active);
        if (n_ignite) atomicAdd(&cs[1], (unsigned long long)n_ignite);
        if (n_items_acc) atomicAdd(&cs[2], (unsigned long long)n_items_acc);
        if (n_phase2) atomicAdd(&cs[4], (unsigned long long)n_phase2);
        if (n_vec_done) atomicAdd(&cs[5], (unsigned long long)n_vec_done);
        if (TEAM && x_steps) {
            atomicAdd(&cs[6], (unsigned long long)x_steps | ((unsigned long long)(one_l2 ? x_steps : 0u) << 32));
            atomicAdd(&cs[7], x_clocks);
        }
    }
    if (TEAM && tn > 1) {
        __syncthreads();
        if (tid == 0) {
            __builtin_amdgcn_fence(__ATOMIC_RELEASE, "agent");
            asm volatile("s_waitcnt vmcnt(0)" ::: "memory");
            const uint32_t before = atomicAdd(&a.xdone[e], 1u);
            const bool last = before == (uint32_t)tn - 1u;
            if (last) __builtin_amdgcn_fence(__ATOMIC_ACQUIRE, "agent");
            ctl[0] = last ? 1u : 0u;
        }
        __syncthreads();
        if (!ctl[0]) {
            if (TEAM == 2) continue;
            return;
        }
    }
    if (a.res_block && !(win_result && !general) && !(a.row_valid && !general && n_steps == 0 && !mit)) {
        __syncthreads();
        wpc.note(36);
        counts_env(g, e, a.status, a.cells, a.tdirty, a.thist, st.running, st.steps, st.elapsed, a.res_block, a.res_elapsed, a.res_sink,
                   reinterpret_cast<int32_t (*)[6]>(vlist + vcap));
        wpc.note(37);
    }
    }
    if (TEAM != 2) return;
    }
}

#ifndef SF_RUN_UNIT
template <int ATT>
__global__ __launch_bounds__(1024) __attribute__((amdgpu_waves_per_eu(8, 8))) void k_win(StepArgs a, const int n_steps_launch)
{
    kernarg_touch<(int)sizeof(StepArgs) + 4>();
    extern __shared__ uint4 s_dyn[];
    const Geo &g = a.g;
    const int tid = threadIdx.x, lane = tid & 63, wave = tid >> 6, n_waves = blockDim.x >> 6;
    const int e = (int)blockIdx.x;
    const unsigned long long clk0 = __builtin_readcyclecounter();
    uint32_t *const wl = reinterpret_cast<uint32_t *>(s_dyn);
    uint32_t *const ctl = wl + (win_lds_bytes(n_waves) + 15) / 16 * 4;
    unsigned long long pre_w = a.vbits[(long long)e * g.vb_env + (tid < g.H ? tid : 0)];
    if (tid >= g.H) pre_w = 0ull;
    EnvState st = a.commit[e];
    int n_steps = n_steps_launch;
    if (!st.running || n_steps < 0) n_steps = 0;
    if (tid < kRunCtl) ctl[tid] = 0;
    const int th_log = 31 - __builtin_clz((unsigned)(g.LR * g.RB));
    uint32_t n_active = 0, n_ignite = 0, n_vec_done = 0;
    bool win_result = false;
    PhaseClock wpc;
    WinEnv we;
    we.cells = a.cells + (long long)e * g.cells_env;
    we.burn = a.burn + (long long)e * g.plane_env;
    we.settled = a.settled ? a.settled + (long long)e * g.plane_env : nullptr;
    we.rtc = a.rtc ? a.rtc + (long long)e * g.rt_env : nullptr;
    we.tdirty = a.tdirty + (long long)e * g.TY * g.TX;
    we.thist = a.thist + (long long)e * g.TY * g.TX * 8;
    we.vb_glob = a.vbits + (long long)e * g.vb_env;
    we.vb_plane = (long long)g.E * g.vb_env;
    we.pre_w = pre_w; we.pre = true; we.hint = 0ull;
    __syncthreads();
    wpc.start();
#ifdef SF_PHASES
    wpc.tl = (e == g_timeline_env && g_timeline_step == -1) ? g_timeline + wave * 64 : nullptr;
#endif
    wpc.note(30);
    const int s_done = run_window<ATT, 0, 0, 1>(a, we, st, n_steps, g.diag != 0, wl, ctl, th_log, n_active, n_ignite, n_vec_done, wpc, e, win_result);
    const bool finished = s_done >= n_steps || !st.running;
    wpc.note(35);
    if (tid == 0) {
        if (s_done > 0) a.commit[e] = st;
        a.todo_out[e] = finished ? 0 : n_steps - s_done;
        if (!finished && a.todo_cnt) a.todo_list[atomicAdd(a.todo_cnt, 1u)] = (uint32_t)e;
        if (blockIdx.x == 0 && a.todo_cnt_next) *a.todo_cnt_next = 0u;
        if (a.cost) {
            const unsigned long long c = (__builtin_readcyclecounter() - clk0) >> 4;
            a.cost[e] = c > 0x0FFFFFFFull ? 0x0FFFFFFFu : (uint32_t)c;
        }
        if (a.counters && s_done) atomicAdd(a.counters + (size_t)((blockIdx.x * 16) & (kCounterShards - 1)) * kCounterRow + 8, (unsigned long long)s_done);
    }
    if (a.counters && lane == 0) {
        unsigned long long *cs = a.counters + (size_t)((blockIdx.x * 16 + wave) & (kCounterShards - 1)) * kCounterRow;
        if (n_active) atomicAdd(&cs[0], (unsigned long long)n_active);
        if (n_ignite) atomicAdd(&cs[1], (unsigned long long)n_ignite);
        if (n_vec_done) atomicAdd(&cs[5], (unsigned long long)n_vec_done);
    }
    if (a.res_block && finished && !win_result) {
        __syncthreads();
        counts_env(g, e, a.status, a.cells, a.tdirty, a.thist, st.running, st.steps, st.elapsed, a.res_block, a.res_elapsed, a.res_sink,
                   reinterpret_cast<int32_t (*)[6]>(wl));
    }
}
#endif

#ifndef SF_RUN_UNIT
__global__ __launch_bounds__(1024) void k_order(int E, const uint32_t *cost, uint32_t *order)
{
    __shared__ uint32_t s_max, s_hist[1024], s_wave[16];
    const int tid = threadIdx.x, lane = tid & 63, wave = tid >> 6;
    if (tid == 0) s_max = 0;
    s_hist[tid] = 0;
    __syncthreads();
    uint32_t mx = 0;
    for (int e = tid; e < E; e += 1024) mx = cost[e] > mx ? cost[e] : mx;
    if (mx) atomicMax(&s_max, mx);
    __syncthreads();
    mx = s_max;
    if (mx == 0) {
        for (int e = tid; e < E; e += 1024) order[e] = (uint32_t)e;
        return;
    }
    const float scale = 1023.0f / (float)mx;
    auto bucket = [&](uint32_t c) { int b = 1023 - (int)((float)c * scale); return b < 0 ? 0 : (b > 1023 ? 1023 : b); };
    for (int e = tid; e < E; e += 1024) atomicAdd(&s_hist[bucket(cost[e])], 1u);
    __syncthreads();
    const uint32_t mine = s_hist[tid];
    const uint32_t incl = wave_scan_incl(mine, lane);
    if (lane == 63) s_wave[wave] = incl;
    __syncthreads();
    uint32_t base = 0;
    for (int w = 0; w < wave; ++w) base += s_wave[w];
    __syncthreads();
    s_hist[tid] = base + incl - mine;
    __syncthreads();
    for (int e = tid; e < E; e += 1024) order[atomicAdd(&s_hist[bucket(cost[e])], 1u)] = (uint32_t)e;
}
#endif

#ifndef SF_RUN_UNIT
__global__ __launch_bounds__(1024) void k_team_plan(int E, int G, int t_min, int t_max, uint32_t ovh, uint32_t floor_c, int scatter, uint32_t *cost, uint32_t *tab, uint32_t *tsize,
                                                    unsigned long long *xg, uint32_t *xdone, int keep_cost, uint32_t *xj, unsigned long long *xcut)
{
    __shared__ uint32_t s_T[1024], s_sum, s_cls[8], s_over;
    const int t = threadIdx.x;
    for (int i = t; i < G; i += 1024) tab[i] = kTeamUnused;
    const uint32_t c = t < E ? cost[t] : 0u;
    for (int i = t; i < E * kTeamMax * 3; i += 1024) xg[i] = 0ull;
    if (t < E) { xdone[t] = 0u; xdone[E + t] = 0u; if (!keep_cost) cost[t] = 0u; }
    if (xj) {
        if (t < E) { xj[t] = 1u; xj[E + t] = 0u; xj[2 * E + 2 + t] = 0xFFFFFFFFu; xcut[t] = 0ull; }
        if (t < 2) xj[2 * E + t] = 0u;
    }
    auto member = [&](int T) -> uint32_t { const uint32_t share = c / (uint32_t)T; return T <= 1 ? c : (share > floor_c ? share : floor_c) + ovh; };
    auto need = [&](uint32_t tgt) -> uint32_t {
        if (t >= E) return 0u;
        if (t_min >= t_max) return (uint32_t)t_min;
        int best = t_min;
        for (int T = t_min; T <= t_max; ++T) {
            if (member(T) <= tgt) return (uint32_t)T;
            if (member(T) < member(best)) best = T;
        }
        return (uint32_t)best;
    };
    auto total = [&](uint32_t v) -> uint32_t {
        __syncthreads();
        if (t == 0) s_sum = 0;
        __syncthreads();
        uint32_t w = v;
        for (int off = 32; off > 0; off >>= 1) w += __shfl_xor(w, off);
        if ((t & 63) == 0 && w) atomicAdd(&s_sum, w);
        __syncthreads();
        return s_sum;
    };
    uint32_t lo = 0, hi = 0;
    if (t_min < t_max) {
        __syncthreads();
        if (t == 0) s_sum = 0;
        __syncthreads();
        if (c) atomicMax(&s_sum, c);
        __syncthreads();
        hi = s_sum;
    }
    for (int it = 0; it < 28 && lo < hi; ++it) {
        const uint32_t mid = lo + (hi - lo) / 2;
        if (total(need(mid)) <= (uint32_t)G) hi = mid; else lo = mid + 1;
    }
    const uint32_t T = need(hi);
    s_T[t] = T;
    if (t < E && tsize) tsize[t] = T;
    if (t < 8) s_cls[t] = 0;
    if (t == 0) s_over = scatter ? 1u : 0u;
    __syncthreads();
    if (t < E) atomicAdd(&s_cls[t & 7], T);
    __syncthreads();
    if (t < 8 && s_cls[t] > (uint32_t)((G - t + 7) / 8)) s_over = 1;
    __syncthreads();
    if (t < E) {
        uint32_t pos = 0;
        if (!s_over) {
            for (int q = t & 7; q < t; q += 8) pos += s_T[q];
            for (uint32_t j = 0; j < T; ++j) tab[(t & 7) + 8 * (pos + j)] = (uint32_t)t | (j << 16) | (T << 24);
        } else {
            for (int q = 0; q < t; ++q) pos += s_T[q];
            for (uint32_t j = 0; j < T; ++j) if (pos + j < (uint32_t)G) tab[pos + j] = (uint32_t)t | (j << 16) | (T << 24);
        }
    }
}
#endif

#ifndef SF_RUN_UNIT
__global__ __launch_bounds__(64) void k_rebuild_vbits(Geo g, const uint8_t *age, unsigned long long *vbits, int env0)
{
    const int w = blockIdx.x, y = blockIdx.y, e = env0 + blockIdx.z, lane = threadIdx.x;
    const int v = w * 64 + lane;
    uint4 r = make_uint4(0, 0, 0, 0);
    if (v < g.PV) r = *reinterpret_cast<const uint4 *>(age + (long long)e * g.age_env + (long long)y * g.P + v * 16);
    const unsigned long long b = __ballot(any4(r) != 0), f = __ballot((r.x & 0xFFu) != 0), l = __ballot((r.w >> 24) != 0);
    if (lane == 0) {
        const long long o = (long long)e * g.vb_env + (long long)y * g.VW + w, plane = (long long)g.E * g.vb_env;
        vbits[o] = b; vbits[plane + o] = f; vbits[2 * plane + o] = l;
    }
}
#endif

#ifndef SF_RUN_UNIT
__global__ __launch_bounds__(64) void k_rm_to_bl(Geo g, const uint8_t *status, const uint8_t *age, uint8_t *cells)
{
    const int v = blockIdx.x * 64 + threadIdx.x, y = blockIdx.y, e = blockIdx.z;
    if (v >= g.PV) return;
    const uint4 m = *reinterpret_cast<const uint4 *>(age + (long long)e * g.age_env + (long long)y * g.P + v * 16);
    const uint4 st = *reinterpret_cast<const uint4 *>(status + (long long)e * g.plane_env + (long long)y * g.P + v * 16);
    uint8_t *row = cells + (long long)e * g.cells_env + bl_vec(g, y, v) + (y & 1) * 16;
    *reinterpret_cast<uint4 *>(row) = m;
    *reinterpret_cast<uint4 *>(row + kBlStatus) = st;
}
#endif
#ifndef SF_RUN_UNIT
__global__ __launch_bounds__(64) void k_bl_to_rm(Geo g, const uint8_t *cells, uint8_t *status, uint8_t *age)
{
    const int v = blockIdx.x * 64 + threadIdx.x, y = blockIdx.y, e = blockIdx.z;
    if (v >= g.PV) return;
    const uint8_t *row = cells + (long long)e * g.cells_env + bl_vec(g, y, v) + (y & 1) * 16;
    if (age) *reinterpret_cast<uint4 *>(age + (long long)e * g.age_env + (long long)y * g.P + v * 16) = *reinterpret_cast<const uint4 *>(row);
    *reinterpret_cast<uint4 *>(status + (long long)e * g.plane_env + (long long)y * g.P + v * 16) = *reinterpret_cast<const uint4 *>(row + kBlStatus);
}
#endif

}
```

### simfire_amd/csrc/simfire_hip.hip

```cpp
#include <emmintrin.h>
#include <hip/hip_runtime.h>

#include <cassert>
#include <cmath>
#include <cstdarg>
#include <cstdint>
#include <cstdio>
#include <cstring>
#include <cstdlib>
#include <algorithm>
#include <map>
#include <string>
#include <tuple>
#include <vector>

#include <dlfcn.h>
#include <rccl/rccl.h>

#include "../../include/simfire_hip.h"
#include "rothermel_dev.h"

#include "sf_common.h"
#include "sf_step_kernels.h"
#include "sf_aux_kernels.h"
// ... 484 lines not shown
    return rc ? rc : finish_call(s, nullptr, !s->async, nullptr);
}

extern "C" int sf_load_fire_map(sf_sim *s, int32_t env, const uint8_t *map)
{
    if (!s || !map) return fail(SF_EINVAL, "sf_load_fire_map: null argument");
    const Geo &g = s->g;
    if (env < 0 || env >= g.E) return fail(SF_EINVAL, "sf_load_fire_map: environment %d out of range", env);
    const size_t n = (size_t)g.H * g.W;
    for (size_t i = 0; i < n; ++i)
        if (map[i] > SF_WETLINE) return fail(SF_EINVAL, "sf_load_fire_map: value %d at cell %zu is not a BurnStatus", map[i], i);
    HIPCHK(hipSetDevice(s->p.device)); LOOP_QUIESCE(s);
    s->fire_rows = 0;
    if (s->delta.snap) s->delta.snap_valid[env] = 0;
    SF_TRY(ensure_stage(s, n));
    dim3 blk(256), grd((g.W + 255) / 256, g.H);
    SF_TRY(ensure_commit(s));
    SF_TRY(ensure_rm(s));
    s->status_fresh = false;
    if (g.att)
        hipLaunchKernelGGL(k_settle_env, grd, blk, 0, s->stream, g, (const uint8_t *)s->status, s->settled, s->burn,
                           (const EnvState *)s->commit, env, 1);
    HIPCHK(hipMemcpyAsync(s->stage, map, n, hipMemcpyHostToDevice, s->stream));
    hipLaunchKernelGGL(k_pack_status, grd, blk, 0, s->stream, g, s->status, s->settled, (const EnvState *)s->commit, env,
                       (const uint8_t *)s->stage);
    HIPCHK(hipGetLastError());
    const int rc = rebuild_tflags(s, env, 1);
    s->tdirty_all = true;
    if (rc) return rc;
    HIPCHK(hipStreamSynchronize(s->stream));
    return SF_OK;
}

static int ensure_rm(sf_sim *s)
{
    if (!s->bl_cur) return SF_OK;
    const Geo &g = s->g;
    hipLaunchKernelGGL(k_bl_to_rm, dim3((g.PV + 63) / 64, g.H, g.E), dim3(64), 0, s->stream, g, (const uint8_t *)s->cells, s->status, s->age);
    HIPCHK(hipGetLastError());
    s->bl_cur = false;
    return SF_OK;
}
static int alloc_bl(sf_sim *s)
{
    if (s->cells_alloc) return SF_OK;
    const Geo &g = s->g;
    const size_t bytes = (size_t)g.E * g.cells_env;
    SF_TRY(dev_alloc(s, &s->cells_alloc, bytes));
    s->cells = s->cells_alloc + (size_t)g.PV * 128;
    HIPCHK(hipMemsetAsync(s->cells_alloc, 0, bytes, s->stream));
    return SF_OK;
}
static bool prefers_bl(const sf_sim *s)
{
    const Geo &g = s->g;
    return g.ab == 1 && !s->generic && (g.VW == 1 || (g.VW == 2 && s->tune.v[SF_TUNE_RUN_TEAM] != 1)) && !s->graph_on && !s->history &&
           (s->fused_mode < 0 || s->fused_mode == 2);
}
static int ensure_rtc(sf_sim *s)
{
    if (s->tables.rtc_valid()) return SF_OK;
    const Geo &g = s->g;
    const size_t n_tab = (size_t)s->tables.size(), tab = (size_t)8 * g.plane_env;
    if (!s->rtc) {
        if (hipMalloc(reinterpret_cast<void **>(&s->rtc), tab * n_tab * sizeof(double)) != hipSuccess) { (void)hipGetLastError(); s->rtc = nullptr; return SF_ENOTSUP; }
        s->bytes += (int64_t)(tab * n_tab * sizeof(double));
    }
    for (size_t i = 0; i < n_tab; ++i)
        if (s->tables[i].rtc_stale)
            hipLaunchKernelGGL(k_rt_cellmajor, dim3((g.P + 255) / 256, g.H), dim3(256), 0, s->stream, g.H, g.P, (const double *)(s->rt + i * tab), s->rtc + i * tab);
    HIPCHK(hipGetLastError());
    s->tables.rtc_built();
    return SF_OK;
}

static int ensure_bl(sf_sim *s)
{
    if (s->bl_cur) return SF_OK;
    const Geo &g = s->g;
    SF_TRY(alloc_bl(s));
    hipLaunchKernelGGL(k_rm_to_bl, dim3((g.PV + 63) / 64, g.H, g.E), dim3(64), 0, s->stream, g, (const uint8_t *)s->status, (const uint8_t *)s->age, s->cells);
    HIPCHK(hipGetLastError());
    s->bl_cur = true;
    return SF_OK;
}

static int ensure_tiles(sf_sim *s)
{
    if (s->tiles_valid) return SF_OK;
    { int rc0 = ensure_rm(s); if (rc0) return rc0; }
    HIPCHK(hipMemsetAsync(s->tflags, 0, s->tflags_bytes, s->stream));
    SF_TRY(rebuild_tflags(s, 0, s->g.E));
    SF_TRY(rebuild_seams(s, 0, s->g.E));
    s->tiles_valid = true;
    return SF_OK;
}
static int ensure_vbits(sf_sim *s)
{
    if (s->vbits_valid) return SF_OK;
    { int rc0 = ensure_rm(s); if (rc0) return rc0; }
    const Geo &g = s->g;
    hipLaunchKernelGGL(k_rebuild_vbits, dim3(g.VW, g.H, g.E), dim3(64), 0, s->stream, g, (const uint8_t *)s->age, s->vbits, 0);
    HIPCHK(hipGetLastError());
    s->vbits_valid = true;
    s->vbits_fl_valid = true;
    return SF_OK;
}

#include "sf_host_views.h"
#include "sf_host_query.h"

extern "C" int sf_last_step_launch(sf_sim *s, int32_t *kind)
{
    if (!s || !kind) return fail(SF_EINVAL, "sf_last_step_launch: null argument");
    *kind = s->last_kind;
    return SF_OK;
}

static RunTable sf_run1_table()
{
    static const RunEntry runs[] = {SF_RUN_ENTRY(1, 0, -1, -1, 0), SF_RUN_ENTRY(1, 0, 1, -1, 0), SF_RUN_ENTRY(1, 1, -1, -1, 0),
                                    SF_RUN_ENTRY(1, 1, 1, -1, 0), SF_RUN_ENTRY(1, 0, 1, 0, 0), SF_RUN_ENTRY(1, 1, 1, 0, 0)};
    return {runs, (int)(sizeof runs / sizeof runs[0]), sizeof(StepArgs)};
}
RunTable sf_run2_table(), sf_run3_table(), sf_run4_table();

enum RunKind { kRunPlain, kRunTeam, kRunJoin, kRunLoop };

static int run_words(int rows, int waves, int vw)
{
    const int need = ((rows + waves * 64 - 1) / (waves * 64)) * vw;
    return need <= 1 ? 1 : (need <= 2 ? 2 : kRunMaxD);
}

static RunKey run_key(const Geo &g, RunKind kind, int words, bool lines)
{
    const int att = g.att ? 1 : 0, diag = g.diag ? 1 : -1;
    switch (kind) {
    case kRunJoin: return {1, att, 1, 0, 2};
    case kRunLoop: return {words, att, -1, -2, 0};
    case kRunTeam: return {words, att, diag, (words == 2 && g.diag && !lines) ? 0 : -1, 1};
    default:
        if (words > 2) return {kRunMaxD, att, -1, -1, 0};
        return {words, att, diag, (g.diag && !lines) ? 0 : -1, 0};
    }
}

static const void *run_fn(const RunKey &k)
{
    static const RunTable tables[] = {sf_run1_table(), sf_run2_table(), sf_run3_table(), sf_run4_table()};
    for (const RunTable &t : tables)
        for (int i = 0; i < t.n; ++i)
            if (t.entries[i].key == k) return t.args_bytes == sizeof(StepArgs) ? t.entries[i].fn : nullptr;
    return nullptr;
}

static hipError_t allow_lds(const sf_sim *s, const void *fn, size_t lds)
{
    if (lds <= 64 * 1024) return hipSuccess;
    auto it = s->lds_allowed.find(fn);
    if (it != s->lds_allowed.end() && it->second >= lds) return hipSuccess;
    const hipError_t e = hipFuncSetAttribute(fn, hipFuncAttributeMaxDynamicSharedMemorySize, (int)lds);
    if (e == hipSuccess) s->lds_allowed[fn] = lds;
    return e;
}

static int launch_resident(sf_sim *s, const void *fn, unsigned grid, unsigned block, size_t lds, void **args)
{
    HIPCHK(allow_lds(s, fn, lds));
    HIPCHK(hipLaunchKernel(fn, dim3(grid), dim3(block), args, lds, s->stream));
    return SF_OK;
}
static int launch_run(sf_sim *s, const RunKey &k, unsigned grid, unsigned block, size_t lds, StepArgs &a, int n_steps, int vcap, int bsz)
{
    const void *fn = run_fn(k);
    if (!fn) return fail(SF_EHIP, "k_run<%d, %d, %d, %d, %d> is not in this library (or its unit was built with another StepArgs)", k.maxd, k.att, k.diag, k.mit, k.team);
    void *args[] = {&a, &n_steps, &vcap, &bsz};
    return launch_resident(s, fn, grid, block, lds, args);
}

static int occupancy(const sf_sim *s, const RunKey &k, unsigned block, size_t lds)
{
    const void *fn = run_fn(k);
    const auto key = std::make_tuple(fn, block, lds);
    auto it = s->occ_cache.find(key);
    if (it != s->occ_cache.end()) return it->second;
    int occ = -1;
    if (!fn || allow_lds(s, fn, lds) != hipSuccess || hipOccupancyMaxActiveBlocksPerMultiprocessor(&occ, fn, (int)block, lds) != hipSuccess) {
        (void)hipGetLastError();
        occ = -1;
    }
    s->occ_cache[key] = occ;
    return occ;
}

struct TeamGeo;
static int team_occupancy(const sf_sim *s, const TeamGeo &t, bool join);
struct TeamGeo { int waves, vcap, rcap, slots, t_min; size_t lds; bool ok; };
static TeamGeo team_geometry(const sf_sim *s)
{
    const Geo &g = s->g;
    TeamGeo t = {};
    const int th = g.LR * g.RB;
    if (g.ab != 1 || g.VW > 2 || g.TY > 64 || g.E > 1024 || g.dense) return t;
    if (g.VW == 1) {
        const bool roomy = g.E * 2 <= s->n_cu && g.H <= 16 * 64;
        t.waves = roomy ? 16 : 8; t.vcap = roomy ? 4096 : 1024; t.rcap = 0; t.t_min = 1;
        if ((g.H + t.waves * 64 - 1) / (t.waves * 64) * g.VW > 2) return t;
    } else {
        t.waves = 16; t.vcap = 2048; t.rcap = 1024 / th * th; t.t_min = (g.H + t.rcap - 1) / t.rcap;
        if (t.rcap < th || (t.rcap + t.waves * 64 - 1) / (t.waves * 64) * g.VW > 2) return t;
    }
    long long all_vec = (long long)g.H * g.PV;
    if (t.vcap > all_vec) t.vcap = (int)((all_vec + 63) / 64 * 64);
    t.lds = run_lds_bytes(g, t.waves, t.vcap, 1, t.rcap);
    if (t.lds > 160 * 1024 || t.t_min > kTeamMax || t.t_min > g.TY) return t;
    int per_cu = (int)((160 * 1024) / t.lds);
    if (per_cu * t.waves > 32) per_cu = 32 / t.waves;
    if (per_cu > 2) per_cu = 2;
    const int occ = team_occupancy(s, t, false);
    if (occ == 0) return t;
    if (occ > 0 && occ < per_cu) per_cu = occ;
    t.slots = s->n_cu * per_cu;
    t.ok = (long long)g.E * t.t_min <= t.slots;
    return t;
}

static int team_occupancy(const sf_sim *s, const TeamGeo &t, bool join)
{
    const unsigned block = (unsigned)t.waves * 64;
    if (join) return occupancy(s, run_key(s->g, kRunJoin, 1, false), block, t.lds);
    const int words = run_words(t.rcap ? t.rcap : s->g.H, t.waves, s->g.VW);
    const int occ = occupancy(s, run_key(s->g, kRunTeam, words, false), block, t.lds);
    const int o2 = occ < 0 ? -1 : occupancy(s, run_key(s->g, kRunTeam, words, true), block, t.lds);
    return (o2 >= 0 && o2 < occ) ? o2 : occ;
}

static TeamGeo join_geometry(const sf_sim *s)
{
    const Geo &g = s->g;
    TeamGeo t = {};
    if (g.ab != 1 || g.VW != 1 || g.TY > 64 || g.H > 16 * 64 || g.E > 1024 || g.E > s->n_cu || g.dense || !g.diag) return t;
    t.waves = 16; t.vcap = 4096; t.rcap = 0; t.t_min = 1;
    const long long all_vec = (long long)g.H * g.PV;
    if (t.vcap > all_vec) t.vcap = (int)((all_vec + 63) / 64 * 64);
    t.lds = run_lds_bytes(g, t.waves, t.vcap, 1, 0);
    if (t.lds > 160 * 1024 || g.TY < 2) return t;
    if (team_occupancy(s, t, true) == 0) return t;
    t.slots = s->n_cu;
    t.ok = true;
    return t;
}
static int team_buffers(sf_sim *s, const TeamGeo &t)
{
    const Geo &g = s->g;
    if (!s->team.tab || s->team.slots < t.slots) {
        if (s->team.tab) { HIPCHK(hipFree(s->team.tab)); s->team.tab = nullptr; }
        SF_TRY(dev_alloc(s, &s->team.tab, (size_t)t.slots));
        s->team.slots = t.slots;
        s->team.plan_ones = 0;
    }
    if (!s->team.xg) {
        SF_TRY(dev_alloc(s, &s->team.xg, (size_t)g.E * kTeamMax * 3));
        SF_TRY(dev_alloc(s, &s->team.xbuf, (size_t)g.E * kTeamMax * 4 * team_xrow(g)));
        SF_TRY(dev_alloc(s, &s->team.xdone, (size_t)2 * g.E + 1));
        HIPCHK(hipMemsetAsync(s->team.xdone, 0, sizeof(uint32_t) * ((size_t)2 * g.E + 1), s->stream));
        SF_TRY(dev_alloc(s, &s->team.size, (size_t)g.E));
        HIPCHK(hipHostMalloc(reinterpret_cast<void **>(&s->team.xerr_pinned), sizeof(uint32_t), hipHostMallocMapped));
        HIPCHK(hipHostGetDevicePointer(reinterpret_cast<void **>(&s->team.xerr_mapped), s->team.xerr_pinned, 0));
        *s->team.xerr_pinned = 0;
        HIPCHK(hipMemsetAsync(s->team.xbuf, 0, (size_t)g.E * kTeamMax * 4 * team_xrow(g), s->stream));
    }
    return SF_OK;
}

static void team_args(const sf_sim *s, StepArgs &a, int rcap, uint32_t *cost)
{
    a.cost = cost;
    a.team_tab = s->team.tab; a.xg = s->team.xg; a.xbuf = s->team.xbuf; a.xdone = s->team.xdone; a.xerr = s->team.xerr_mapped;
    a.xrow = team_xrow(s->g); a.team_rcap = rcap;
    a.team_far = s->tune.v[SF_TUNE_TEAM_PLACEMENT] == 2;
    a.order = nullptr;
}

static int launch_k_run_join(sf_sim *s, StepArgs &a, int n_steps, const TeamGeo &t, bool eager)
{
    const Geo &g = s->g;
    SF_TRY(team_buffers(s, t));
    if (!s->team.xj) {
        SF_TRY(dev_alloc(s, &s->team.xj, (size_t)3 * g.E + 2));
        SF_TRY(dev_alloc(s, &s->team.xcut, (size_t)g.E));
        SF_TRY(dev_alloc(s, &s->team.jlog, (size_t)1 + 3 * kJoinLog));
    }
    HIPCHK(hipMemsetAsync(s->team.jlog, 0, sizeof(uint32_t), s->stream));
    s->team.jlog_valid = true;
    hipLaunchKernelGGL(k_team_plan, dim3(1), dim3(1024), 0, s->stream, g.E, t.slots, 1, 1, 0u, 0u, 1, s->run_cost, s->team.tab, s->team.size, s->team.xg, s->team.xdone, 0,
                       s->team.xj, s->team.xcut);
    s->team.plan_ones = 0;
    team_args(s, a, 0, s->run_cost);
    a.xj = s->team.xj; a.xcut = s->team.xcut; a.tsize = s->team.size; a.jlog = s->team.jlog;
    const int place = s->tune.v[SF_TUNE_TEAM_PLACEMENT];
    a.join_local = place == 1 ? 0 : (place == 2 ? 2 : 1);
    a.join_floor = eager ? 0 : 12000; a.join_ovh = eager ? 0 : (a.join_local == 1 ? 3000 : 12000);
    return launch_run(s, run_key(g, kRunJoin, 1, false), (unsigned)t.slots, (unsigned)t.waves * 64, t.lds, a, n_steps, t.vcap, 64);
}


static int launch_k_run_team(sf_sim *s, StepArgs &a, int n_steps, const TeamGeo &t, int t_min, int t_max, int steps_before, bool keep_cost = false)
{
    const Geo &g = s->g;
    SF_TRY(team_buffers(s, t));
    const uint32_t ovh = (uint32_t)((long long)(steps_before > 0 ? steps_before : 0) * 6500 / 16);
    const uint32_t floor_c = (uint32_t)((long long)(steps_before > 0 ? steps_before : 0) * 12000 / 16);
    const int scatter = s->tune.v[SF_TUNE_TEAM_PLACEMENT] == 1 ? 1 : 0;
    const long long ones_key = (t_min == 1 && t_max == 1) ? 1 + (long long)scatter + 2ll * t.slots + ((long long)g.E << 32) : 0;
    if (!ones_key || s->team.plan_ones != ones_key)
        hipLaunchKernelGGL(k_team_plan, dim3(1), dim3(1024), 0, s->stream, g.E, t.slots, t_min, t_max, ovh, floor_c, scatter,
                           s->run_cost, s->team.tab, s->team.size, s->team.xg, s->team.xdone, keep_cost ? 1 : 0, (uint32_t *)nullptr, (unsigned long long *)nullptr);
    s->team.plan_ones = ones_key;
    team_args(s, a, t.rcap, keep_cost ? nullptr : s->run_cost);
    const int words = run_words(t.rcap ? t.rcap : g.H, t.waves, g.VW);
    return launch_run(s, run_key(g, kRunTeam, words, a.mit != nullptr), (unsigned)t.slots, (unsigned)t.waves * 64, t.lds, a, n_steps, t.vcap, 64);
}

struct StepPlan {
    bool generic, fused;
    int nw, vcap, bsz;
    size_t lds;
    int win;
    bool result;
    TeamGeo tgeo, jgeo;
    bool team_forced, team_wide, team_auto;
    bool win_first;
    bool win_only;
    bool balance;
    bool team_any, team_segments;
};

static void plan_modes(const sf_sim *s, StepPlan &p, int n_steps)
{
    const int seg_knob = s->tune.v[SF_TUNE_RUN_SEGMENT];
    p.balance = seg_knob > 0 && s->g.E > s->n_cu * (p.nw <= 8 ? 2 : 1) && !p.win_first;
    p.team_any = (p.team_forced || p.team_wide || p.team_auto) && p.bsz == 64 && !p.win_first;
    p.team_segments = p.team_any && seg_knob > 0 && !p.balance;
    p.win_only = false;
    if (p.win_first) {
        const int F = s->fire_rows, wv = (F + 14) / 16 + 1;
        const int room = wv > 3 ? 0 : std::min((64 - F) / 2, 32 - 8 * wv);
        p.win_only = n_steps + 1 <= room && p.win == 1;
    }
}

static StepPlan plan_step(const sf_sim *s, int n_steps, bool lines)
{
    StepPlan p = {};
    const Geo &g = s->g;
    const Tuning &tn = s->tune;
    const bool polled = n_steps == 1 && !lines && !s->last_was_step1 && s->step1_polls >= 2;
    const long long n_wave_tiles = (long long)g.E * g.TY * g.TX;
    p.fused = s->fused_mode == 1 || (s->fused_mode < 0 && n_wave_tiles <= 12288);
    p.generic = g.ab > 1 || s->generic;
    p.win = tn.v[SF_TUNE_RUN_WINDOW] < 0 ? 0 : tn.v[SF_TUNE_RUN_WINDOW];
    if (!p.generic && !(s->graph_on && s->parents) && !s->history && s->fused_mode != 0 && s->fused_mode != 1) {
        const int waves_knob = tn.v[SF_TUNE_RUN_WAVES], envs_knob = tn.v[SF_TUNE_RUN_MIN_ENVS], vcap_knob = tn.v[SF_TUNE_RUN_VCAP];
        int nw = waves_knob < 1 ? 1 : (waves_knob > 16 ? 16 : waves_knob);
        const int need = (g.H + 63) / 64;
        if (nw > need) nw = need;
        const int min_nw = (int)(((long long)g.H * g.VW + 64 * kRunMaxD - 1) / (64 * kRunMaxD));
        if (nw < min_nw) nw = min_nw;
        long long all_vec = (long long)g.H * g.PV;
        int vcap = vcap_knob < 64 ? 64 : vcap_knob;
        if (vcap > all_vec) vcap = (int)((all_vec + 63) / 64 * 64);
        size_t lds = run_lds_bytes(g, nw, vcap);
        p.win_first = p.win != 0 && tn.v[SF_TUNE_RUN_COMPACT] != 0 && (g.E > s->n_cu || tn.v[SF_TUNE_RUN_COMPACT] == 2) && !lines && g.VW == 1 &&
                      g.H >= 64 && g.H <= 1024 && g.PV >= 4 && !g.dense && s->fire_rows > 0 && s->fire_rows <= 62 && n_steps <= 64 && !tn.set[SF_TUNE_RUN_WAVES] &&
                      g.diag && (tn.v[SF_TUNE_RUN_TEAM] == 0 || tn.v[SF_TUNE_RUN_TEAM] == 1) && s->fused_mode != 2;
        const bool all_young = tn.v[SF_TUNE_RUN_WINDOW] != 0 && s->fire_rows > 0 && s->fire_rows + 2LL * n_steps <= 60;
        if (tn.v[SF_TUNE_RUN_COMPACT] && g.E > s->n_cu && nw > 8 && min_nw <= 8 && !tn.set[SF_TUNE_RUN_WAVES] && !all_young) {
            const int vcap2 = vcap > 1024 ? 1024 : vcap;
            const size_t lds2 = run_lds_bytes(g, 8, vcap2);
            if (lds2 <= 80 * 1024) { nw = 8; vcap = vcap2; lds = lds2; }
        }
        const bool fits = nw <= 16 && g.W <= 4096 && g.H <= 65535 && g.VW <= kRunMaxD && lds <= 160 * 1024;
        p.tgeo = team_geometry(s);
        p.jgeo = join_geometry(s);
        const int team_knob = tn.v[SF_TUNE_RUN_TEAM];
        p.team_forced = p.tgeo.ok && team_knob >= 2 && team_knob <= kTeamMax && team_knob <= g.TY && team_knob >= p.tgeo.t_min && (long long)g.E * team_knob <= p.tgeo.slots;
        if (lines && p.tgeo.rcap > 0 && (long long)team_knob * p.tgeo.rcap < g.H) p.team_forced = false;
        p.team_wide = p.tgeo.ok && team_knob != 1 && g.VW == 2 && !lines;
        const bool wanted = s->fused_mode == 2 || ((n_steps >= 2 || lines || polled) && (g.VW == 1 || p.team_wide) && g.E >= envs_knob);
        p.team_auto = p.tgeo.ok && g.VW == 1 && g.E < p.tgeo.slots && (team_knob == -1 || (team_knob == 0 && g.E >= 2 && g.E * 4 <= s->n_cu && p.tgeo.waves == 16));
        if (fits && wanted) { p.nw = nw; p.vcap = vcap; p.lds = lds; }
    }
    const int bsz_knob = tn.v[SF_TUNE_RUN_BATCH];
    p.bsz = bsz_knob < 8 ? 8 : (bsz_knob > 64 ? 64 : bsz_knob);
    p.result = tn.v[SF_TUNE_RUN_RESULT] != 0;
    plan_modes(s, p, n_steps);
    return p;
}

struct Segment {
    int n;
    int recut;
    bool join, team;
    bool windows;
    int t_min, t_max;
    int team_max;
};

static Segment plan_segment(const sf_sim *s, const StepPlan &p, int n_steps, int done, bool lines)
{
    const Geo &g = s->g;
    const Tuning &tn = s->tune;
    const TeamGeo &tgeo = p.tgeo;
    const int seg_knob = tn.v[SF_TUNE_RUN_SEGMENT];
    Segment sg = {};
    sg.n = p.balance && n_steps - done > seg_knob + seg_knob / 2 ? seg_knob : n_steps - done;
    const int tseg = (p.team_wide || p.team_auto) && !p.team_forced ? 2 * seg_knob : seg_knob;
    const int tk = tn.v[SF_TUNE_RUN_TEAM];
    const bool team_fixed = p.team_segments && tn.v[SF_TUNE_TEAM_RECUT] != 0 && !(tgeo.rcap > 0 && tk == -1) &&
                            (long long)tgeo.t_min * (tgeo.rcap ? tgeo.rcap : g.H) >= g.H &&
                            (p.team_forced || (p.team_wide && tgeo.slots - (long long)g.E * tgeo.t_min < (g.E + 3) / 4));
    if (p.team_segments && !team_fixed && n_steps - done > tseg + tseg / 2) sg.n = tseg;
    sg.recut = team_fixed ? (p.team_forced ? 2 * seg_knob : tseg) : 0;
    bool young = false;
    if (p.team_wide && !p.team_forced && tk == 0 && tgeo.rcap > 0 && s->fire_rows > 0) {
        const long long room = (long long)tgeo.rcap - s->fire_rows - 2LL * done - 7LL * g.LR * g.RB - 2;
        const long long fit = room / 2;
        if (done == 0 && fit >= n_steps && s->fire_rows + 2LL * n_steps <= 480) { young = true; sg.n = n_steps - done; sg.recut = 0; }
    }
    const int join_knob = tn.v[SF_TUNE_RUN_JOIN];
    const int join_min = join_knob > 1 ? join_knob : (join_knob < -1 ? -join_knob : 192);
    sg.join = !p.win_first && join_knob != 0 && !p.team_forced && !p.team_wide && ((g.E >= 2 && !tn.set[SF_TUNE_RUN_TEAM]) || tn.set[SF_TUNE_RUN_JOIN]) && !p.balance && !lines && p.bsz == 64 && done == 0 &&
              n_steps >= join_min && !tn.set[SF_TUNE_RUN_WAVES] && !tn.set[SF_TUNE_RUN_VCAP] && p.jgeo.ok;
    if (sg.join) { sg.n = n_steps; sg.recut = seg_knob >= 4 ? seg_knob / 2 : 2; sg.team_max = kTeamMax; }
    sg.team = !p.win_first && !sg.join && p.team_any && !p.balance && (p.team_forced || p.team_wide || (s->cost_steps > 0 && n_steps - done >= seg_knob / 2));
    if (sg.team) {
        sg.team_max = p.team_forced ? tk : (kTeamMax < g.TY ? kTeamMax : g.TY);
        sg.windows = tgeo.rcap > 0 && !p.team_forced && tk == -1;
        sg.t_min = young ? 1 : (p.team_forced ? tk : (sg.windows ? 1 : tgeo.t_min));
        sg.t_max = young ? 1 : (team_fixed && !p.team_forced ? tgeo.t_min : sg.team_max);
    }
    return sg;
}

static StepArgs handle_args(const sf_sim *s)
{
    StepArgs a;
    memset(&a, 0, sizeof a);
    a.g = s->g; a.status = s->status; a.age = s->age; a.cells = s->cells; a.burn = s->burn; a.rt = s->rt;
    a.commit = s->commit; a.tmp = s->tmp; a.flags = s->flags; a.tflags = s->tflags; a.tile_list = s->tile_list;
    a.n_active = s->n_active; a.seam = s->seam; a.settled = s->settled; a.tdirty = s->tdirty; a.thist = s->thist; a.vbits = s->vbits;
    a.launch = 0; a.from_commit = 1; a.ring = s->ring;
    return a;
}

static int run_resident(sf_sim *s, const StepPlan &p, StepArgs &a, int n_steps, bool row_was_fresh)
{
    const Geo &g = s->g;
    const int32_t *mit_dev = a.mit;
    const int mit_k = a.mit_k;
    if (p.result) {
        if (s->tdirty_all) HIPCHK(hipMemsetAsync(s->tdirty, 1, s->n_tiles_max, s->stream));
        s->tdirty_all = false;
    }
    a.cost = s->run_cost;
    s->last_team_max = 0;
    if (p.win_first) {
        const size_t wlds = (win_lds_bytes(16) + 15) / 16 * 16 + kRunCtl * 4;
        a.todo_out = s->todo; a.order = nullptr;
        a.row_valid = (row_was_fresh && p.result) ? 1 : 0;
        if (!s->todo_cnt) { int rc0 = dev_alloc(s, &s->todo_cnt, (size_t)16); if (rc0) return rc0; HIPCHK(hipMemsetAsync(s->todo_cnt, 0, 16 * sizeof(uint32_t), s->stream)); }
        a.todo_cnt = s->todo_cnt + (s->win_seq & 1); a.todo_cnt_next = s->todo_cnt + ((s->win_seq + 1) & 1); a.todo_list = s->run_order;
        s->win_seq++;
        if (p.result) { a.res_block = s->status_block; a.res_elapsed = s->elapsed_dev; a.res_sink = s->sink; }
        const void *wk = g.att ? reinterpret_cast<const void *>(k_win<1>) : reinterpret_cast<const void *>(k_win<0>);
        void *args[] = {&a, &n_steps};
        { int rc0 = launch_resident(s, wk, (unsigned)g.E, 1024, wlds, args); if (rc0) return rc0; }
        a.todo_out = nullptr; a.res_block = nullptr; a.res_elapsed = nullptr; a.res_sink = nullptr;
        s->last_launches++;
        a.todo = s->todo; a.todo_skip = 1;
    }
    for (int done = 0; done < n_steps && !p.win_only;) {
        const Segment sg = plan_segment(s, p, n_steps, done, mit_dev != nullptr);
        a.team_recut = sg.recut;
        if (p.balance) {
            hipLaunchKernelGGL(k_order, dim3(1), dim3(1024), 0, s->stream, g.E, (const uint32_t *)s->run_cost, s->run_order);
            a.order = s->run_order;
        }
        a.mit = mit_dev ? mit_dev + (size_t)done * g.E * mit_k * 3 : nullptr;
        if (p.result && done + sg.n == n_steps) { a.res_block = s->status_block; a.res_elapsed = s->elapsed_dev; a.res_sink = s->sink; }
        a.row_valid = (row_was_fresh && done == 0 && !p.win_first && p.result) ? 1 : 0;
        if (sg.join) {
            int rc0 = launch_k_run_join(s, a, sg.n, p.jgeo, s->tune.v[SF_TUNE_RUN_JOIN] < 0);
            if (rc0) return rc0;
        } else if (sg.team) {
            a.todo = nullptr; a.todo_out = sg.windows ? s->todo : nullptr;
            int rc0 = launch_k_run_team(s, a, sg.n, p.tgeo, sg.t_min, sg.t_max, s->cost_steps);
            if (rc0) return rc0;
            if (sg.windows) {
                a.todo = s->todo; a.todo_out = nullptr; a.row_valid = 0;
                rc0 = launch_k_run_team(s, a, sg.n, p.tgeo, p.tgeo.t_min, p.tgeo.t_min, 0, true);
                if (rc0) return rc0;
                a.todo = nullptr;
            }
            a.cost = s->run_cost;
        } else {
            int rc0 = launch_run(s, run_key(g, kRunPlain, run_words(g.H, p.nw, g.VW), a.mit != nullptr), (unsigned)g.E, (unsigned)p.nw * 64, p.lds, a,
                                 sg.n, p.vcap, p.bsz);
            if (rc0) return rc0;
            if (g.VW > 1) s->vbits_fl_valid = false;
        }
        if (sg.join || sg.team) s->last_team_max = sg.team_max;
        s->cost_steps = sg.n;
        done += sg.n;
        s->last_launches++;
    }
    if (p.win_only) s->cost_steps = n_steps;
    s->status_fresh = p.result;
    s->tiles_valid = false;
    s->last_kind = p.win_first ? 4 : 2;
    return SF_OK;
}

static int enqueue_steps(sf_sim *s, StepPlan p, int n_steps, const int32_t *mit_dev, int mit_k, hipEvent_t t0)
{
    const Geo &g = s->g;
    const Tuning &tn = s->tune;
    const bool row_was_fresh = s->status_fresh;
    s->status_fresh = false;
    s->last_launches = 0;
    const int n_requested = n_steps;
    if (n_steps != 1 || mit_dev || s->last_was_step1) s->step1_polls = 0;
    if (p.nw) {
        int rc0 = ensure_commit(s);
        if (rc0) return rc0;
        if ((p.team_forced || p.team_wide || p.team_auto) && !s->vbits_fl_valid) s->vbits_valid = false;
        rc0 = ensure_vbits(s);
        if (rc0) return rc0;
        rc0 = ensure_bl(s);
        if (rc0) return rc0;
        if (p.win) {
            rc0 = ensure_rtc(s);
            if (rc0 == SF_ENOTSUP) { p.win = 0; p.win_first = false; plan_modes(s, p, n_steps); }
            else if (rc0) return rc0;
        }
    } else if (!p.generic) {
        int rc0 = ensure_tiles(s);
        if (rc0) return rc0;
    }
    if (!p.nw) { int rc0 = ensure_rm(s); if (rc0) return rc0; }
    StepArgs a = handle_args(s);
    a.counters = s->counters_on ? s->counters : nullptr;
    a.parents = s->graph_on ? s->parents : nullptr;
    a.team_timeout = 100000ull * (unsigned long long)(tn.v[SF_TUNE_TEAM_TIMEOUT_MS] == 0 ? 2000 : (tn.v[SF_TUNE_TEAM_TIMEOUT_MS] < 1 ? 1 : tn.v[SF_TUNE_TEAM_TIMEOUT_MS]));
    a.team_start_timeout = tn.v[SF_TUNE_TEAM_TIMEOUT_MS] == 0 ? 0ull : a.team_timeout;
    a.mit = mit_dev; a.mit_k = mit_k;
    a.win = p.win;
    if (p.nw && p.win) { a.rtc = s->rtc; a.win_hint = s->win_hint; }
    if (t0) HIPCHK(hipEventRecord(t0, s->stream));
    if (p.nw) {
        int rc0 = run_resident(s, p, a, n_steps, row_was_fresh);
        if (rc0) return rc0;
        n_steps = 0;
    } else if (n_steps > 0) {
        s->vbits_valid = false;
        if (p.generic) s->tiles_valid = false;
        s->last_kind = p.generic ? 3 : (p.fused ? 1 : 0);
    }
    const long long n_wave_tiles = (long long)g.E * g.TY * g.TX;
    const dim3 sel_grid((unsigned)((n_wave_tiles + kSelectThreads - 1) / kSelectThreads));
    const int waves_per_cu = tn.v[SF_TUNE_WAVES_PER_CU];
    long long want = p.fused ? (n_wave_tiles + kWaves - 1) / kWaves : (long long)s->n_cu * waves_per_cu / kWaves;
    if (!p.fused && want * kWaves > n_wave_tiles) want = (n_wave_tiles + kWaves - 1) / kWaves;
    const dim3 step_grid((unsigned)(want < 1 ? 1 : want));
    const StepKernel kern = pick_step_kernel(g.RB, p.fused);
    const dim3 cell_grid((unsigned)((g.W + 255) / 256), (unsigned)g.H, (unsigned)g.E);
    for (int i = 0; i < n_steps; ++i) {
        a.launch = s->seq;
        a.from_commit = s->committed ? 1 : 0;
        a.ring = s->ring;
        if (p.generic) {
            if (g.ab == 1) hipLaunchKernelGGL(k_step_cells<uint8_t>, cell_grid, dim3(256), 0, s->stream, a);
            else if (g.ab == 2) hipLaunchKernelGGL(k_step_cells<uint16_t>, cell_grid, dim3(256), 0, s->stream, a);
            else hipLaunchKernelGGL(k_step_cells<uint32_t>, cell_grid, dim3(256), 0, s->stream, a);
        } else {
            if (!p.fused) hipLaunchKernelGGL(k_select, sel_grid, dim3(kSelectThreads), 0, s->stream, a);
            hipLaunchKernelGGL(kern, step_grid, dim3(kWaves * 64), (size_t)kWaves * g.lds_wave_bytes, s->stream, a);
            s->ring ^= 1;
        }
        if (a.parents) {
            if (p.generic || p.fused) hipLaunchKernelGGL(k_graph_pass, cell_grid, dim3(256), 0, s->stream, a);
            else hipLaunchKernelGGL(k_graph_pass_tiles, dim3((unsigned)(s->n_cu * 8)), dim3(256), 0, s->stream, a);
        }
        if (s->history) hipLaunchKernelGGL(k_record, cell_grid, dim3(256), 0, s->stream, g, (const uint8_t *)s->status,
                                           (const EnvState *)(s->tmp + (size_t)(a.launch & 1) * g.E), s->history, s->history_cap);
        s->seq = (s->seq + 1) % 6;
        s->committed = false;
    }
    if (s->fire_rows > 0) { const long long fr = (long long)s->fire_rows + 2LL * n_requested; s->fire_rows = fr > g.H ? g.H : (int)fr; }
    s->last_was_step1 = n_requested == 1 && !mit_dev;
    return SF_OK;
}

static int enqueue_call(sf_sim *s, const StepPlan &p, int n_steps, const int32_t *mit_dev, int mit_k, bool hold, hipEvent_t t0)
{
    if (!s->wind.sched.empty()) {
// ... 645 lines not shown
```

### simfire_amd/csrc/simfire_hip_run2.hip

```cpp
#define SF_RUN_UNIT 1
#include <hip/hip_runtime.h>

#include "../../include/simfire_hip.h"
#include "sf_common.h"
#include "sf_step_kernels.h"
#include "sf_aux_kernels.h"
#include "sf_run_kernels.h"
#include "sf_run_table.h"

RunTable sf_run2_table()
{
    static const RunEntry runs[] = {
        SF_RUN_ENTRY(1, 0, -1, -1, 1), SF_RUN_ENTRY(1, 0, 1, -1, 1), SF_RUN_ENTRY(1, 1, -1, -1, 1), SF_RUN_ENTRY(1, 1, 1, -1, 1),
        SF_RUN_ENTRY(1, 0, 1, 0, 2), SF_RUN_ENTRY(1, 1, 1, 0, 2),
        SF_RUN_ENTRY(1, 0, -1, -2, 0), SF_RUN_ENTRY(1, 1, -1, -2, 0)};
    return {runs, (int)(sizeof runs / sizeof runs[0]), sizeof(StepArgs)};
}
```

Measured before the change: 24140 billion.

## Specialize join-team run kernel: drop stats, split kernarg access, unroll batch loop

Adds a TEAM==3 variant that keeps statistics counters, so the default TEAM==2 join kernel (MAXD1, ATT0, DIAG1, MIT0) can compile out per-batch stat accumulation. The host dispatches to the counted variant only when counters are requested. It also reads hot fields from kernarg memory while keeping the by-value copy for geometry, and lets a single-round deal skip the atomic grab. It enables the two-buffer prefetch path for the lean grow kernel. The aim is to cut VGPR pressure, register moves and LDS atomics in the hot batch loop, at the cost of an extra kernel instantiation and more compile-time variants.

```diff
diff --git a/profiles/isa_step_path.py b/profiles/isa_step_path.py
--- /dev/null
+++ b/profiles/isa_step_path.py
@@ -0,0 +1,171 @@
+#!/usr/bin/env python3
+import argparse
+import os
+import re
+import sys
+import tempfile
+
+sys.path.insert(0, os.path.dirname(os.path.abspath(__file__)))
+import isa_waits as iw
+
+BLOCK = re.compile(r"^(?:\.L(BB\d+_\d+):|; %bb\.\d+:)")
+IN_LOOP = re.compile(r"in Loop: Header=(BB\d+_\d+) Depth=(\d+)")
+PARENT = re.compile(r"Parent Loop (BB\d+_\d+) Depth=(\d+)")
+IS_HEADER = re.compile(r"This (?:Inner )?Loop Header: Depth=(\d+)")
+CLASSES = ("VALU", "SALU", "LDS", "VMEM", "SMEM", "lane", "wait", "branch", "other")
+
+
+def kernel_text(asm_text, args):
+    key = iw.mangled(args)
+    lines = asm_text.splitlines()
+    start = next((i for i, ln in enumerate(lines) if key in ln and re.match(r"^_Z\S+:", ln)), None)
+    if start is None:
+        raise LookupError("no k_run<%s> in this assembly" % args)
+    end = next(i for i in range(start, len(lines)) if lines[i].startswith(".Lfunc_end"))
+    return lines[start + 1:end], lines[start].split(":")[0]
+
+
+def resources(asm_text, symbol):
+    lines = asm_text.splitlines()
+    out = {}
+    at = next(i for i, ln in enumerate(lines) if ln.startswith(symbol + ":"))
+    for ln in lines[at:]:
+        m = re.match(r"^; (NumVgprs|ScratchSize|Occupancy): (\d+)", ln)
+        if m:
+            out[m.group(1)] = int(m.group(2))
+            if m.group(1) == "Occupancy":
+                break
+    name = next(i for i, ln in enumerate(lines) if re.match(r"^\s+\.name:\s+%s\s*$" % re.escape(symbol), ln))
+    lo = next(i for i in range(name, -1, -1) if lines[i].startswith("  - ."))
+    hi = next((i for i in range(name + 1, len(lines)) if lines[i].startswith("  - .") or not lines[i].startswith(" ")), len(lines))
+    for ln in lines[lo:hi]:
+        m = re.match(r"^\s+\.(sgpr_spill_count|vgpr_spill_count|vgpr_count|private_segment_fixed_size):\s+(\d+)", ln)
+        if m:
+            out[m.group(1)] = int(m.group(2))
+    return out
+
+
+def blocks(raw):
+    out, cur = [], None
+    for ln in raw:
+        if BLOCK.match(ln):
+            cur = {"label": BLOCK.match(ln).group(1), "notes": [ln], "ins": []}
+            out.append(cur)
+        elif cur is None:
+            continue
+        elif ln.lstrip().startswith(";"):
+            if not cur["ins"]:
+                cur["notes"].append(ln)
+        elif ln.strip() and not ln.lstrip().startswith("."):
+            cur["ins"].append(iw.instr(ln))
+    for b in out:
+        notes = " ".join(b["notes"])
+        b["parents"] = [m.group(1) for m in PARENT.finditer(notes)]
+        b["header"] = b["label"] if IS_HEADER.search(notes) else None
+        m = IN_LOOP.search(notes)
+        b["inner"] = b["header"] or (m.group(1) if m else None)
+    parents = {b["header"]: b["parents"] for b in out if b["header"]}
+    for b in out:
+        b["chain"] = (parents.get(b["inner"], []) + [b["inner"]]) if b["inner"] else []
+    return out
+
+
+def classify(op):
+    name = op.split()[0]
+    if name in ("v_readlane_b32", "v_writelane_b32"):
+        return "lane"
+    if name.startswith("s_waitcnt"):
+        return "wait"
+    if name.startswith(("s_cbranch", "s_branch", "s_endpgm", "s_setpc", "s_barrier")):
+        return "branch"
+    if name.startswith(("s_load", "s_buffer_load", "s_memtime", "s_memrealtime")):
+        return "SMEM"
+    if name.startswith("ds_"):
+        return "LDS"
+    if name.startswith(("global_", "flat_", "buffer_", "scratch_")):
+        return "VMEM"
+    if name.startswith("v_"):
+        return "VALU"
+    if name.startswith("s_"):
+        return "SALU"
+    return "other"
+
+
+def count(bs):
+    c = dict.fromkeys(CLASSES, 0)
+    for b in bs:
+        for op in b["ins"]:
+            c[classify(op)] += 1
+    c["all"] = sum(c[k] for k in CLASSES)
+    return c
+
+
+def header_moves(body):
+    load, dpp = iw.find_prefetch(body)
+    first, _, hdr = iw.loop_range(body, dpp)
+    n64 = n32 = nw = run = best = 0
+    for i in range(first, load - 3):
+        op = iw.instr(body[i])
+        if op.startswith(("v_mov_b64", "v_mov_b32")) and re.match(r"v_mov_b(64|32)(_e32)? v(\d+|\[\d+:\d+\]), v", op):
+            n64 += op.startswith("v_mov_b64")
+            n32 += op.startswith("v_mov_b32")
+            run += 1
+            best = max(best, run)
+        elif not iw.LABEL.match(body[i]):
+            run = 0
+        if op.startswith("s_waitcnt") and "vmcnt" in op:
+            nw += 1
+    return {"v_mov_b64": n64, "v_mov_b32": n32, "vmcnt_waits": nw, "longest_run": best, "header": hdr, "span": load - 3 - first}
+
+
+def analyse(asm_text, args):
+    raw, symbol = kernel_text(asm_text, args)
+    body = iw.kernel_lines(asm_text, args)
+    res = resources(asm_text, symbol)
+    hm = header_moves(body)
+    bs = blocks(raw)
+    batch_hdr = hm["header"]
+    chain = next(b["chain"] for b in bs if b["header"] == batch_hdr)
+    step_hdr = chain[-3] if len(chain) >= 3 else chain[0]
+    in_batch = [b for b in bs if batch_hdr in b["chain"]]
+    in_step = [b for b in bs if step_hdr in b["chain"] and batch_hdr not in b["chain"]]
+    entry = [b for b in bs if not b["chain"]]
+    return {"resources": res, "header_moves": hm, "batch_loop": count(in_batch), "step_outside": count(in_step), "outside_loops": count(entry),
+            "batch_header": batch_hdr, "step_header": step_hdr}
+
+
+def report(asm_text, args, label="", out=sys.stdout):
+    a = analyse(asm_text, args)
+    r, hm = a["resources"], a["header_moves"]
+    p = lambda *x: print(*x, file=out)
+    p("# k_run<%s>%s" % (args.replace(",", ", "), ("  [%s]" % label) if label else ""))
+    p("registers: %d VGPRs, %d spilled SGPRs, %d spilled VGPRs, scratch %d B per lane, %d waves per SIMD" %
+      (r.get("NumVgprs", r.get("vgpr_count", -1)), r.get("sgpr_spill_count", -1), r.get("vgpr_spill_count", -1),
+       r.get("ScratchSize", r.get("private_segment_fixed_size", -1)), r.get("Occupancy", -1)))
+    p("loops: steps %s, batches %s" % (a["step_header"], a["batch_header"]))
+    p("%-28s | %5s | %s" % ("static instructions", "all", " | ".join("%5s" % k for k in CLASSES)))
+    for name, key in (("batch loop (with the walk)", "batch_loop"), ("step loop outside it", "step_outside"), ("outside the step loop", "outside_loops")):
+        c = a[key]
+        p("%-28s | %5d | %s" % (name, c["all"], " | ".join("%5d" % c[k] for k in CLASSES)))
+    p("head of the batch loop, %d instructions in front of the prefetch: %d v_mov_b64 + %d v_mov_b32 (longest run %d), %d waits that name vmcnt" %
+      (hm["span"], hm["v_mov_b64"], hm["v_mov_b32"], hm["longest_run"], hm["vmcnt_waits"]))
+    return a
+
+
+def main():
+    ap = argparse.ArgumentParser(description=__doc__.split("\n")[0])
+    ap.add_argument("--unit", default="simfire_hip_run2.hip")
+    ap.add_argument("--kernel", default="1,0,1,0,2", help="template arguments of k_run: MAXD,ATT,DIAG,MIT,TEAM")
+    ap.add_argument("--asm", default=None)
+    ap.add_argument("--label", default="")
+    a = ap.parse_args()
+    if a.asm:
+        text = open(a.asm).read()
+    else:
+        with tempfile.TemporaryDirectory() as d:
+            text = open(iw.compile_asm(a.unit, os.path.join(d, "unit.s"))).read()
+    report(text, a.kernel, a.label)
+
+
+if __name__ == "__main__":
+    main()
diff --git a/simfire_amd/csrc/sf_run_kernels.h b/simfire_amd/csrc/sf_run_kernels.h
--- a/simfire_amd/csrc/sf_run_kernels.h
+++ b/simfire_amd/csrc/sf_run_kernels.h
@@ -66,12 +66,11 @@
 };
 
 template <int ATT, int CNT = 0>
-__device__ __forceinline__ WalkAcc run_walk(const StepArgs &a, const RunEnv &ev, const Masks &mk, int complete,
+__device__ __forceinline__ WalkAcc run_walk(const Geo &g, const RunEnv &ev, const Masks &mk, int complete,
                                             uint32_t lo_mask, uint32_t hi_mask, const uint32_t *strips,
                                             uint32_t pend, int lane, int th_log, PhaseClock &pc,
                                             uint32_t excl, uint32_t w16, uint4 s7)
 {
-    const Geo &g = a.g;
     WalkAcc acc = {0u, 0u, 0u, 0u};
     auto front = [&](uint32_t j, int own) {
         WalkCell c;
@@ -309,21 +308,33 @@
 template <int MAXD, int ATT, int DIAG, int MIT, int TEAM = 0>
 __global__ __launch_bounds__(1024) void k_run(StepArgs a_by_value, const int n_steps_launch, int vcap, int bsz)
 {
+    constexpr bool kGrow = TEAM >= 2;
+#if defined(SF_PHASES) || defined(SF_NO_LEAN_STATS)
+    constexpr bool kStats = true;
+#else
+    constexpr bool kStats = !(MAXD == 1 && ATT == 0 && DIAG == 1 && MIT == 0 && TEAM == 2);
+#endif
     kernarg_touch<(int)sizeof(StepArgs) + 12>();
 #ifdef SF_ARGS_BY_VALUE
     constexpr bool kArgsByValue = true;
+    constexpr bool kArgsSplit = false;
+#elif defined(SF_NO_ARGS_SPLIT)
+    constexpr bool kArgsByValue = kGrow || MIT == -2 || (MIT == 0 && TEAM == 0) || (TEAM == 1 && MAXD == 2);
+    constexpr bool kArgsSplit = false;
 #else
-    constexpr bool kArgsByValue = TEAM == 2 || MIT == -2 || (MIT == 0 && TEAM == 0) || (TEAM == 1 && MAXD == 2);
+    constexpr bool kArgsByValue = MIT == -2 || (MIT == 0 && TEAM == 0) || (TEAM == 1 && MAXD == 2);
+    constexpr bool kArgsSplit = kGrow;
 #endif
     const StepArgs &a = kArgsByValue ? a_by_value : *(const StepArgs *)__builtin_amdgcn_kernarg_segment_ptr();
+    const StepArgs &ah = kArgsSplit ? a_by_value : a;
     extern __shared__ uint4 s_dyn[];
-    const Geo &g = a.g;
+    const Geo &g = ah.g;
     const int tid = threadIdx.x, wave = tid >> 6, lane = tid & 63, n_waves = blockDim.x >> 6, nthr = blockDim.x;
     int e_ = 0, tm_ = 0, tn_ = 1;
     bool no_work = false;
     if (TEAM) {
         const uint32_t tt = a.team_tab[blockIdx.x];
-        if (tt == kTeamUnused) { if (TEAM != 2) return; no_work = true; }
+        if (tt == kTeamUnused) { if (!kGrow) return; no_work = true; }
         else { e_ = (int)(tt & 0xFFFFu); tm_ = (int)((tt >> 16) & 0xFFu); tn_ = (int)(tt >> 24); }
     } else if (a.todo_cnt) {
         const uint32_t n_left = *a.todo_cnt;
@@ -332,7 +343,7 @@
     } else e_ = a.order ? (int)a.order[blockIdx.x] : (int)blockIdx.x;
     int j_s0 = -1;
     for (bool first_pass = true;; first_pass = false) {
-    if (TEAM == 2 && (!first_pass || no_work)) {
+    if (kGrow && (!first_pass || no_work)) {
         if (a.team_recut >= n_steps_launch) return;
         uint32_t *sc = reinterpret_cast<uint32_t *>(s_dyn);
         JoinArgs ja;
@@ -365,7 +376,7 @@
     uint32_t *tcnt = reinterpret_cast<uint32_t *>(halo + 2 * g.PV);
 
     constexpr bool kWinPre = (MIT == 0 || MIT == -1) && MAXD == 1 && TEAM == 0;
-    constexpr bool kWinAny = ((MIT == 0 && MAXD <= 2) || (MIT == -1 && MAXD == 1 && TEAM == 0 && DIAG == 1)) && TEAM != 2;
+    constexpr bool kWinAny = ((MIT == 0 && MAXD <= 2) || (MIT == -1 && MAXD == 1 && TEAM == 0 && DIAG == 1)) && !kGrow;
     constexpr bool kWinAdvice = kWinAny && !(MAXD == 1 && TEAM == 0);
     unsigned long long pre_w = 0ull, hint_v = 0ull;
     int32_t todo_v = 0;
@@ -401,7 +412,7 @@
     if (tid < kRunCtl) ctl[tid] = 0;
     const int th_log = 31 - __builtin_clz((unsigned)(g.LR * g.RB));
     uint32_t n_active = 0, n_ignite = 0, n_items_acc = 0, n_phase2 = 0, n_vec_done = 0;
-    constexpr bool kWin = ((MIT == 0 && MAXD <= 2) || (MIT == -1 && MAXD == 1 && TEAM == 0 && DIAG == 1)) && TEAM != 2;
+    constexpr bool kWin = ((MIT == 0 && MAXD <= 2) || (MIT == -1 && MAXD == 1 && TEAM == 0 && DIAG == 1)) && !kGrow;
     constexpr int kWinGen = (MAXD == 1 && TEAM == 0) ? 0 : 1;
     constexpr int kWinMit = MIT == -1 ? 1 : 0;
     int32_t px = 0, py = 0, pty = 0;
@@ -434,7 +445,7 @@
         if (a.counters && tid == 0 && s_begin)
             atomicAdd(a.counters + (size_t)((blockIdx.x * 16) & (kCounterShards - 1)) * kCounterRow + 8, (unsigned long long)s_begin);
     }
-    if (TEAM == 2 && j_s0 >= 0) s_begin = j_s0;
+    if (kGrow && j_s0 >= 0) s_begin = j_s0;
     const bool general = !kWin || (TEAM && tn > 1) || (s_begin < n_steps && (st.running || mit));
     if (TEAM == 0 && kWin && MIT == 0 && !general) {
 #ifdef SF_PHASES
@@ -528,10 +539,10 @@
         }
     }
     bool has_up = TEAM && tm > 0, has_dn = TEAM && tm + 1 < tn;
-    if (TEAM == 2 && tm == 0 && j_s0 < 0 && tid == 0)
+    if (kGrow && tm == 0 && j_s0 < 0 && tid == 0)
         __hip_atomic_store(a.xj + 2 * g.E + 2 + e, (uint32_t)__builtin_amdgcn_s_getreg((20 << 0) | (0 << 6) | (31 << 11)) & 15u, __ATOMIC_RELAXED, __HIP_MEMORY_SCOPE_AGENT);
     auto team_release = [&]() {
-        if (TEAM == 2 && a.join_local == 1) asm volatile("s_waitcnt vmcnt(0)" ::: "memory");
+        if (kGrow && a.join_local == 1) asm volatile("s_waitcnt vmcnt(0)" ::: "memory");
         else __builtin_amdgcn_fence(__ATOMIC_RELEASE, "agent");
     };
     auto team_acquire = [&]() { __builtin_amdgcn_fence(__ATOMIC_ACQUIRE, "agent"); };
@@ -640,8 +651,8 @@
         }
     }
     if (TEAM && tn > 1) {
-        if (wave == 0) line_up(TEAM == 2 && j_s0 >= 0 ? 2u + (uint32_t)(j_s0 / a.team_recut) : 1u, TEAM == 2 && j_s0 >= 0);
-        if (TEAM == 2) __syncthreads();
+        if (wave == 0) line_up(kGrow && j_s0 >= 0 ? 2u + (uint32_t)(j_s0 / a.team_recut) : 1u, kGrow && j_s0 >= 0);
+        if (kGrow) __syncthreads();
     }
 
     RunEnv ev;
@@ -1030,11 +1041,17 @@
             pc.mark(2);
 
             struct VecIn { uint32_t item; uint4 up, mid, dn, sr; uint32_t l0, l1, l2, r0, r1, r2; };
-            const bool dealt = n_waves == 16 && n_chunk <= 2u * (uint32_t)bsz;
+#ifdef SF_NO_ONE_ROUND
+            const bool one_round = n_waves == 16 && n_chunk <= 2u * (uint32_t)bsz;
+            const uint32_t grab_off = one_round ? (uint32_t)(n_waves * bsz) : 0u;
+#else
+            const bool one_round = n_waves == 16 && n_chunk <= (uint32_t)(n_waves * bsz);
+            constexpr uint32_t grab_off = 0u;
+#endif
             auto grab = [&]() {
                 uint32_t j = 0;
                 if (lane == 0) j = atomicAdd(&ctl[6 + k], (uint32_t)bsz);
-                return (uint32_t)__builtin_amdgcn_readfirstlane((int)j) + (dealt ? (uint32_t)(n_waves * bsz) : 0u);
+                return (uint32_t)__builtin_amdgcn_readfirstlane((int)j) + grab_off;
             };
             auto fetch = [&](uint32_t j0, VecIn &in) {
                 const bool has = lane < bsz && j0 + lane < n_chunk;
@@ -1061,13 +1078,24 @@
                     if (diag) { in.r1 = *reinterpret_cast<const uint32_t *>(p_up + 128); in.r2 = *reinterpret_cast<const uint32_t *>(p_dn + 128); }
                 }
             };
-            const uint32_t j_first = dealt ? (uint32_t)(wave * bsz) : grab();
+            const uint32_t j_first = one_round ? (kGrow ? (uint32_t)__builtin_amdgcn_readfirstlane(wave * bsz) : (uint32_t)(wave * bsz)) : grab();
             pc.note(16);
+#ifdef SF_NO_UNROLL_TEAM2
+            constexpr bool kTwoSets = TEAM == 0 && MAXD == 1;
+#else
+            constexpr bool kTwoSets = (TEAM == 0 || (kGrow && !kStats)) && MAXD == 1;
+#endif
             VecIn vin_a, vin_b;
             if (j_first < n_chunk) fetch(j_first, vin_a);
             pc.note(17);
             auto batch = [&](const VecIn &cur, const uint32_t j0, VecIn &nxt, uint32_t &j_next) __attribute__((always_inline)) {
+#ifdef SF_NO_ONE_ROUND
                 j_next = j0 + (uint32_t)bsz < n_chunk ? grab() : n_chunk;
+#else
+                j_next = !one_round && j0 + (uint32_t)bsz < n_chunk ? grab() : n_chunk;
+#endif
+                if (kGrow && kTwoSets)
+                    asm volatile("" :: "v"(cur.mid.x), "v"(cur.sr.x), "v"(cur.up.x), "v"(cur.dn.x), "v"(cur.l0), "v"(cur.l1), "v"(cur.l2), "v"(cur.r0), "v"(cur.r1), "v"(cur.r2));
                 pc.note(18);
                 constexpr bool kEarly = !(TEAM && MAXD == 2);
                 if (kEarly && j_next < n_chunk) fetch(j_next, nxt);
@@ -1100,7 +1128,7 @@
                 }
                 const uint32_t item_l = (uint32_t)__builtin_amdgcn_update_dpp(-1, (int)item, 0x138, 0xF, 0xF, false);
                 const uint32_t item_r = (uint32_t)__builtin_amdgcn_update_dpp(-1, (int)item, 0x130, 0xF, 0xF, false);
-                n_vec_done += (lane == 0) ? (n_chunk - j0 < (uint32_t)bsz ? n_chunk - j0 : (uint32_t)bsz) : 0u;
+                if (kStats) n_vec_done += (lane == 0) ? (n_chunk - j0 < (uint32_t)bsz ? n_chunk - j0 : (uint32_t)bsz) : 0u;
                 const uint4 midL = and4(mid, L4);
                 const uint4 vsrc = and4(or4(up, dn), L4);
                 const uint4 hsrc = diag ? or4(midL, vsrc) : midL;
@@ -1222,20 +1250,18 @@
                     __builtin_amdgcn_wave_barrier();
                     __builtin_amdgcn_fence(__ATOMIC_ACQUIRE, "wavefront");
                     pc.mark(6);
-                    const WalkAcc wk = run_walk<ATT, loop ? 1 : 0>(a, ev, mk, st.complete, lo_mask, hi_mask, strips, total, lane, th_log, pc, excl, m16 | (line16 << 16), s7n);
-                    n_active += wk.n_active;
-                    n_ignite += wk.n_ignite;
+                    const WalkAcc wk = run_walk<ATT, loop ? 1 : 0>(g, ev, mk, st.complete, lo_mask, hi_mask, strips, total, lane, th_log, pc, excl, m16 | (line16 << 16), s7n);
+                    if (kStats) { n_active += wk.n_active; n_ignite += wk.n_ignite; }
                     if (loop && wk.n_ignite && lane == 0) { atomicAdd(ev.tot + SF_UNBURNED, -(int32_t)wk.n_ignite); atomicAdd(ev.tot + SF_BURNING, (int32_t)wk.n_ignite); }
                     if (wk.cand && lane == 0) reinterpret_cast<uint8_t *>(ctl + 3 + k)[1] = 1;
-                    n_items_acc += (lane == 0) ? total : 0u;
-                    n_phase2++;
+                    if (kStats) { n_items_acc += (lane == 0) ? total : 0u; n_phase2++; }
                 } else {
                     __builtin_amdgcn_wave_barrier();
                 }
                 pc.mark(10);
                 if (!kEarly && j_next < n_chunk) fetch(j_next, nxt);
             };
-            if (TEAM == 0 && MAXD == 1) {
+            if (kTwoSets) {
                 for (uint32_t ja = j_first; ja < n_chunk;) {
                     uint32_t jb;
                     batch(vin_a, ja, vin_b, jb);
@@ -1256,16 +1282,16 @@
         if (TEAM && tn > 1) asm volatile("s_waitcnt vmcnt(0)" ::: "memory");
         __syncthreads();
         pc.mark(0);
-        const bool cut_step = TEAM && a.team_recut > 0 && (s + 1) % a.team_recut == 0 && s + 1 < n_steps;
+        const bool cut_step = TEAM && ah.team_recut > 0 && (s + 1) % ah.team_recut == 0 && s + 1 < n_steps;
         const bool recut_now = cut_step && tn > 1;
         int tn_new = tn;
-        if (TEAM == 2 && cut_step) {
+        if (kGrow && cut_step) {
             if (tm == 0 && tid == 0) {
                 const uint32_t c = __hip_atomic_load(a.xj + e, __ATOMIC_RELAXED, __HIP_MEMORY_SCOPE_AGENT) & 0xFFu;
                 const uint32_t t_cap = (uint32_t)(kTeamMax < g.TY ? kTeamMax : g.TY);
                 ctl[20] = c > t_cap ? t_cap : (c < (uint32_t)tn ? (uint32_t)tn : c);
                 const unsigned long long now = __builtin_readcyclecounter();
-                long long per = (long long)((now - join_clk) / (unsigned long long)a.team_recut);
+                long long per = (long long)((now - join_clk) / (unsigned long long)ah.team_recut);
                 join_clk = now;
                 if (tn > 1) per = (per - a.join_ovh) * tn;
                 if (per < a.join_floor) per = a.join_floor;
@@ -1280,19 +1306,19 @@
             team_release();
             __syncthreads();
         }
-        if (TEAM == 2 && cut_step && tm == 0) tn_new = __builtin_amdgcn_readfirstlane((int)ctl[20]);
+        if (kGrow && cut_step && tm == 0) tn_new = __builtin_amdgcn_readfirstlane((int)ctl[20]);
         if (TEAM && tn > 1) {
             if (wave == 0) {
                 typedef unsigned long long u64;
                 int lane = threadIdx.x & 63;
                 asm volatile("" : "+v"(lane));
-                const unsigned long long xt0 = a.counters ? __builtin_readcyclecounter() : 0ull;
+                const unsigned long long xt0 = kStats && a.counters ? __builtin_readcyclecounter() : 0ull;
                 const uint32_t epoch = (uint32_t)s + 1u, par = (uint32_t)s & 1u;
-                uint8_t *xb_me = a.xbuf + ((size_t)(e * kTeamMax + tm) * 4) * (size_t)a.xrow;
+                uint8_t *xb_me = ah.xbuf + ((size_t)(e * kTeamMax + tm) * 4) * (size_t)ah.xrow;
                 for (int side = 0; side < 2 && !one_l2; ++side) {
                     if (!(side ? has_dn : has_up)) continue;
                     const int yb = side ? R1 - 1 : R0;
-                    u64 *dst = reinterpret_cast<u64 *>(xb_me + (size_t)(side * 2 + par) * a.xrow);
+                    u64 *dst = reinterpret_cast<u64 *>(xb_me + (size_t)(side * 2 + par) * ah.xrow);
                     for (int v = lane; v < g.PV; v += 64)
                         if ((vb[yb * VW + (v >> 6)] >> (v & 63)) & 1ull) {
                             const uint4 val = *reinterpret_cast<const uint4 *>(ev.cells + bl_vec(g, yb, v) + (yb & 1) * 16);
@@ -1311,15 +1337,15 @@
                 }
                 asm volatile("s_waitcnt vmcnt(0)" ::: "memory");
                 if (lane == 0) {
-                    const u64 gv = ((u64)epoch << 32) | (u64)(ctl[3 + k] & 0xFFFFu) | (TEAM == 2 ? (u64)tn_new << 16 : 0ull);
-                    if (one_l2) __hip_atomic_store(a.xg + ((size_t)e * kTeamMax + tm) * 3 + par, gv, __ATOMIC_RELAXED, __HIP_MEMORY_SCOPE_WORKGROUP);
-                    else __hip_atomic_store(a.xg + ((size_t)e * kTeamMax + tm) * 3 + par, gv, __ATOMIC_RELAXED, __HIP_MEMORY_SCOPE_AGENT);
+                    const u64 gv = ((u64)epoch << 32) | (u64)(ctl[3 + k] & 0xFFFFu) | (kGrow ? (u64)tn_new << 16 : 0ull);
+                    if (one_l2) __hip_atomic_store(ah.xg + ((size_t)e * kTeamMax + tm) * 3 + par, gv, __ATOMIC_RELAXED, __HIP_MEMORY_SCOPE_WORKGROUP);
+                    else __hip_atomic_store(ah.xg + ((size_t)e * kTeamMax + tm) * 3 + par, gv, __ATOMIC_RELAXED, __HIP_MEMORY_SCOPE_AGENT);
                 }
                 u64 x = (u64)epoch << 32;
                 {
                     const unsigned long long t0 = __builtin_amdgcn_s_memrealtime();
                     for (;;) {
-                        if (lane < tn) x = __hip_atomic_load(a.xg + ((size_t)e * kTeamMax + lane) * 3 + par, __ATOMIC_RELAXED, __HIP_MEMORY_SCOPE_AGENT);
+                        if (lane < tn) x = __hip_atomic_load(ah.xg + ((size_t)e * kTeamMax + lane) * 3 + par, __ATOMIC_RELAXED, __HIP_MEMORY_SCOPE_AGENT);
                         if (__all((uint32_t)(x >> 32) == epoch)) break;
                         __builtin_amdgcn_s_sleep(1);
                         if (gave_up || __builtin_amdgcn_s_memrealtime() - t0 > a.team_timeout) {
@@ -1331,7 +1357,7 @@
                 }
                 const bool live_any = __ballot(lane < tn && (x & 0xFFull)) != 0ull, cand_any = __ballot(lane < tn && (x & 0xFF00ull)) != 0ull;
                 if (lane == 0) ctl[3 + k] = (live_any ? FLAG_LIVE : 0u) | (cand_any ? FLAG_CAND : 0u);
-                if (TEAM == 2 && cut_step && lane == 0) ctl[20] = (uint32_t)(x >> 16) & 0xFFu;
+                if (kGrow && cut_step && lane == 0) ctl[20] = (uint32_t)(x >> 16) & 0xFFu;
                 for (int side = 0; side < 2 && one_l2; ++side) {
                     if (!(side ? has_dn : has_up)) continue;
                     const int yh = side ? R1 : R0 - 1;
@@ -1351,7 +1377,7 @@
                 for (int side = 0; side < 2 && !one_l2; ++side) {
                     if (!(side ? has_dn : has_up)) continue;
                     const int nj = side ? tm + 1 : tm - 1, yh = side ? R1 : R0 - 1;
-                    const u64 *src = reinterpret_cast<const u64 *>(a.xbuf + ((size_t)(e * kTeamMax + nj) * 4 + (size_t)((side ^ 1) * 2 + par)) * a.xrow);
+                    const u64 *src = reinterpret_cast<const u64 *>(ah.xbuf + ((size_t)(e * kTeamMax + nj) * 4 + (size_t)((side ^ 1) * 2 + par)) * ah.xrow);
                     u64 word = 0;
                     if (lane < 3 * VW) word = __hip_atomic_load(src + lane, __ATOMIC_RELAXED, __HIP_MEMORY_SCOPE_AGENT);
                     for (int v0 = 0; v0 < g.PV; v0 += 64) {
@@ -1374,7 +1400,7 @@
                         (which == 0 ? vb : (which == 1 ? vf : vl))[yh * VW + w] = word;
                     }
                 }
-                if (a.counters && lane == 0) { x_clocks += __builtin_readcyclecounter() - xt0; x_steps++; }
+                if (kStats && a.counters && lane == 0) { x_clocks += __builtin_readcyclecounter() - xt0; x_steps++; }
             }
             __builtin_amdgcn_fence(__ATOMIC_RELEASE, "workgroup", "local");
             __builtin_amdgcn_s_barrier();
@@ -1386,15 +1412,15 @@
         st.complete = __builtin_amdgcn_readfirstlane(st.complete);
         st.time_quit = __builtin_amdgcn_readfirstlane(st.time_quit);
         if (loop) loop_finish();
-        if (TEAM == 2 && cut_step && tn > 1) tn_new = __builtin_amdgcn_readfirstlane((int)ctl[20]);
-        if (TEAM == 2 && gave_up) tn_new = tn;
+        if (kGrow && cut_step && tn > 1) tn_new = __builtin_amdgcn_readfirstlane((int)ctl[20]);
+        if (kGrow && gave_up) tn_new = tn;
         if ((recut_now || tn_new > tn) && (st.running || mit)) {
-            if (TEAM == 2 && tn == 1) {
+            if (kGrow && tn == 1) {
                 store_band();
                 team_release();
                 __syncthreads();
             }
-            if (TEAM == 2 && tn_new > tn && tm == 0 && tid == 0) {
+            if (kGrow && tn_new > tn && tm == 0 && tid == 0) {
                 a.commit[e] = st;
                 team_release();
                 __hip_atomic_store(a.xcut + e, ((unsigned long long)tn_new << 24) | (unsigned long long)(s + 1), __ATOMIC_RELAXED, __HIP_MEMORY_SCOPE_AGENT);
@@ -1403,19 +1429,19 @@
                 if (li < (uint32_t)kJoinLog) { a.jlog[1 + 3 * li] = (uint32_t)e; a.jlog[2 + 3 * li] = (uint32_t)(s + 1); a.jlog[3 + 3 * li] = (uint32_t)tn_new; }
             }
             team_acquire();
-            if (TEAM == 2) { tn = tn_new; has_up = tm > 0; has_dn = tm + 1 < tn; }
+            if (kGrow) { tn = tn_new; has_up = tm > 0; has_dn = tm + 1 < tn; }
             const int left = n_steps - (s + 1);
-            cut_bands(a.team_recut < left ? a.team_recut : left);
+            cut_bands(ah.team_recut < left ? ah.team_recut : left);
             load_band();
             ev.vb = vb; ev.vf = vf; ev.vl = vl;
             rpt = (R1 - R0 + nthr - 1) / nthr;
             row0 = R0;
             __syncthreads();
-            if (wave == 0) line_up(2u + (uint32_t)((s + 1) / a.team_recut), true);
+            if (wave == 0) line_up(2u + (uint32_t)((s + 1) / ah.team_recut), true);
             __syncthreads();
         }
     }
-    if (TEAM == 2 && tm == 0 && tid == 0) {
+    if (kGrow && tm == 0 && tid == 0) {
         atomicOr(a.xj + e, kJoinClosed);
         __hip_atomic_store(a.xcut + e, ~0ull, __ATOMIC_RELAXED, __HIP_MEMORY_SCOPE_AGENT);
         __hip_atomic_store(a.xj + g.E + e, 0u, __ATOMIC_RELAXED, __HIP_MEMORY_SCOPE_AGENT);
@@ -1456,7 +1482,7 @@
             }
     }
     wpc.note(49);
-    if (a.counters && lane == 0) {
+    if (kStats && a.counters && lane == 0) {
         int cw = wave;
         asm volatile("" : "+v"(cw));
         unsigned long long *cs = a.counters + (size_t)((blockIdx.x * 16 + cw) & (kCounterShards - 1)) * kCounterRow;
@@ -1482,7 +1508,7 @@
         }
         __syncthreads();
         if (!ctl[0]) {
-            if (TEAM == 2) continue;
+            if (kGrow) continue;
             return;
         }
     }
@@ -1494,7 +1520,7 @@
         wpc.note(37);
     }
     }
-    if (TEAM != 2) return;
+    if (!kGrow) return;
     }
 }
 
diff --git a/simfire_amd/csrc/simfire_hip.hip b/simfire_amd/csrc/simfire_hip.hip
--- a/simfire_amd/csrc/simfire_hip.hip
+++ b/simfire_amd/csrc/simfire_hip.hip
@@ -810,7 +810,10 @@
     const int place = s->tune.v[SF_TUNE_TEAM_PLACEMENT];
     a.join_local = place == 1 ? 0 : (place == 2 ? 2 : 1);
     a.join_floor = eager ? 0 : 12000; a.join_ovh = eager ? 0 : (a.join_local == 1 ? 3000 : 12000);
-    return launch_run(s, run_key(g, kRunJoin, 1, false), (unsigned)t.slots, (unsigned)t.waves * 64, t.lds, a, n_steps, t.vcap, 64);
+    RunKey key = run_key(g, kRunJoin, 1, false), counted = key;
+    counted.team = 3;
+    if (a.counters && run_fn(counted)) key = counted;
+    return launch_run(s, key, (unsigned)t.slots, (unsigned)t.waves * 64, t.lds, a, n_steps, t.vcap, 64);
 }
 
 
diff --git a/simfire_amd/csrc/simfire_hip_run2.hip b/simfire_amd/csrc/simfire_hip_run2.hip
--- a/simfire_amd/csrc/simfire_hip_run2.hip
+++ b/simfire_amd/csrc/simfire_hip_run2.hip
@@ -12,7 +12,7 @@
 {
     static const RunEntry runs[] = {
         SF_RUN_ENTRY(1, 0, -1, -1, 1), SF_RUN_ENTRY(1, 0, 1, -1, 1), SF_RUN_ENTRY(1, 1, -1, -1, 1), SF_RUN_ENTRY(1, 1, 1, -1, 1),
-        SF_RUN_ENTRY(1, 0, 1, 0, 2), SF_RUN_ENTRY(1, 1, 1, 0, 2),
+        SF_RUN_ENTRY(1, 0, 1, 0, 2), SF_RUN_ENTRY(1, 0, 1, 0, 3), SF_RUN_ENTRY(1, 1, 1, 0, 2),
         SF_RUN_ENTRY(1, 0, -1, -2, 0), SF_RUN_ENTRY(1, 1, -1, -2, 0)};
     return {runs, (int)(sizeof runs / sizeof runs[0]), sizeof(StepArgs)};
 }
```

Result: faster. 25030 billion (median of 6 runs) (+3.7%).
